# YooSungHyun/RNNTransducer

Hardware: AMD Instinct MI355X
Metric: utterances/sec (higher is better)
Workload: dtype f32

## Files before the change

### include/rnnt_hip.h

```cpp
#ifndef RNNT_HIP_H_
#define RNNT_HIP_H_

#include <stddef.h>
#include <stdint.h>

#ifdef __cplusplus
extern "C" {
#endif

#define RNNT_HIP_ABI_VERSION 4

#define RNNT_OK 0
#define RNNT_ERR_INVALID (-1)
#define RNNT_ERR_LAUNCH (-2)
#define RNNT_ERR_UNSUPPORTED (-3)
#define RNNT_ERR_TIMEOUT (-4)

int rnnt_hip_version(void);
const char* rnnt_hip_last_error(void);
int rnnt_hip_device_cus(void);

enum {
  RNNT_K_GEMM = 0,
  RNNT_K_LSTM_FWD = 1,
  RNNT_K_LSTM_BWD = 2,
  RNNT_K_LSE = 3,
  RNNT_K_ALPHABETA = 4,
  RNNT_K_LATGRAD = 5,
  RNNT_K_MISC = 6,
  RNNT_K_GEMM_HP = 7,
  RNNT_K_HP_SPLIT = 8,
  RNNT_K_COUNT = 9
};
int rnnt_hip_prof_enable(int on);
int rnnt_hip_prof_collect(double* ms, double* work, int64_t* count, int nkinds);

int rnnt_hip_lstm_launch_log_enable(int on);
int64_t rnnt_hip_lstm_launch_log(char* buf, size_t n);

#define RNNT_GEMM_GELU_A 1u
#define RNNT_GEMM_GELU_B 2u
#define RNNT_GEMM_ACCUM 4u
#define RNNT_GEMM_MUL_DGELU 8u
#define RNNT_GEMM_EXACT_F32 16u
#define RNNT_GEMM_HP_F16 32u

typedef struct rnnt_gemm_desc {
  int64_t M, N, K;
  const float* A;
  int64_t a_div, a_so, a_si, a_sk;
  int32_t a_mc;
  const int64_t* a_rowidx;
  const float* B;
  int64_t b_sn, b_sk;
  float* C;
  int64_t c_div, c_so, c_si;
  const float* bias;
  const float* aux;
  uint32_t flags;
  void* workspace;
  size_t workspace_bytes;
} rnnt_gemm_desc;

size_t rnnt_hip_gemm_workspace_bytes(int64_t M, int64_t N, int64_t K);
int rnnt_hip_gemm_f32(const rnnt_gemm_desc* d, void* stream);

size_t rnnt_hip_hp_bytes(int64_t rows, int64_t K);
int rnnt_hip_hp_split(const float* x, int64_t rows, int64_t K, int64_t ld, int32_t transpose, int64_t src_rows, int64_t shift,
                      void* planes, uint32_t* amax, int32_t amax_given, void* stream);
int rnnt_hip_hp_split_both(const float* x, int64_t M, int64_t C, int64_t ld, const uint32_t* rowmax, const uint32_t* colmax,
                           void* planes_rm, void* planes_t, void* stream);
size_t rnnt_hip_gemm_hp_workspace_bytes(int64_t M, int64_t N, int64_t K);
int rnnt_hip_gemm_hp(const void* A, const uint32_t* a_amax, const void* B, const uint32_t* b_amax, int64_t M, int64_t N, int64_t K,
                     float* C, int64_t ldc, const float* bias, uint32_t flags, void* workspace, size_t workspace_bytes,
                     void* stream);

typedef struct rnnt_hp_problem {
  const void* A; const uint32_t* a_amax;
  const void* B; const uint32_t* b_amax;
  int64_t M, N, K;
  float* C; int64_t ldc;
  uint32_t flags;
} rnnt_hp_problem;
size_t rnnt_hip_gemm_hp_grouped_workspace_bytes(const rnnt_hp_problem* problems, int32_t n);
int rnnt_hip_gemm_hp_grouped(const rnnt_hp_problem* problems, int32_t n, uint32_t xcd_skip, void* workspace, size_t workspace_bytes,
                             void* stream);

#define RNNT_CELL_LSTM 0
#define RNNT_CELL_GRU 1
#define RNNT_CELL_RNN_TANH 2
#define RNNT_CELL_RNN_RELU 3

typedef struct rnnt_lstm_desc {
  int32_t T, B, I, H, D;
  int32_t cell;
  const int32_t* lens;
  const float* x;
  int64_t x_st, x_sb;
  const float* w_ih[2];
  const float* w_hh[2];
  const float* b_ih[2];
  const float* b_hh[2];
  float* y;
  float* y_drop;
  float dropout_p;
  uint64_t dropout_seed;
  float* gates;
  float* cst;
  float* aux;
  void* workspace;
  size_t workspace_bytes;
  uint32_t* status;
  float x_abs_bound;
  const int32_t* row_idx;
  int32_t n_rows;
} rnnt_lstm_desc;

size_t rnnt_hip_lstm_workspace_bytes(int32_t T, int32_t B, int32_t I, int32_t H, int32_t D);
int32_t rnnt_hip_lstm_max_batch(int32_t H, int32_t D, int32_t cell);
int32_t rnnt_hip_lstm_free_xcds(int32_t T, int32_t B, int32_t H, int32_t D, int32_t cell);
int32_t rnnt_hip_lstm_takes_row_idx(int32_t T, int32_t B, int32_t I, int32_t H, int32_t D, int32_t cell);
int rnnt_hip_lstm_fwd(const rnnt_lstm_desc* d, void* stream);

#define RNNT_PRECISION_FP32 0
#define RNNT_PRECISION_F16 1
int rnnt_hip_lstm_fwd_ex(const rnnt_lstm_desc* d, uint32_t precision, void* stream);
int32_t rnnt_hip_lstm_takes_f16(int32_t T, int32_t B, int32_t I, int32_t H, int32_t D, int32_t cell);

typedef struct rnnt_lstm_bwd_desc {
  rnnt_lstm_desc f;
  const float* dy;
  float* dx;
  float* dw_ih[2];
  float* dw_hh[2];
  float* db[2];
  float* db_hh[2];
  int32_t accumulate;
  int32_t phase;
  int32_t beside_recurrence;
} rnnt_lstm_bwd_desc;
#define RNNT_LSTM_BWD_ALL 0
#define RNNT_LSTM_BWD_RECUR 1
#define RNNT_LSTM_BWD_WEIGHTS 2

int rnnt_hip_lstm_bwd(const rnnt_lstm_bwd_desc* d, void* stream);
int rnnt_hip_lstm_bwd_ex(const rnnt_lstm_bwd_desc* d, uint32_t precision, void* stream);
int rnnt_hip_lstm_check(const void* workspace, void* stream);
int rnnt_hip_lstm_debug_read(const void* workspace, int32_t T, int32_t B, int32_t I, int32_t H, int32_t D,
                             uint64_t* out, int32_t nwg, void* stream);

size_t rnnt_hip_joint_loss_workspace_bytes(int32_t B, int32_t T, int32_t U1, int32_t V);
int rnnt_hip_joint_loss_fwd_bwd(const float* A, int64_t a_sb, int64_t a_st, const float* C, int64_t c_sb, int64_t c_su,
                                const float* bias, const int32_t* labels, const int32_t* t_lens,
                                const int32_t* u_lens, int32_t B, int32_t T, int32_t U1, int32_t V, int32_t blank,
                                float gscale, float* nll, float* dA, float* dC, void* workspace,
                                size_t workspace_bytes, void* stream);

int rnnt_hip_joint_loss_bwd(const float* A, int64_t a_sb, int64_t a_st, const float* C, int64_t c_sb, int64_t c_su,
                            const float* bias, const int32_t* labels, const int32_t* t_lens, const int32_t* u_lens,
                            int32_t B, int32_t T, int32_t U1, int32_t V, int32_t blank, float gscale, const float* gvec,
                            int32_t gvec_stride, float* dA, float* dC, void* workspace, size_t workspace_bytes, void* stream);
int rnnt_hip_scaled_sum_f32(const float* x, int32_t n, float scale, float* out, void* stream);

int rnnt_hip_joint_logits_fwd(const float* A, int64_t a_sb, int64_t a_st, const float* C, int64_t c_sb, int64_t c_su,
                              const float* bias, int32_t B, int32_t T, int32_t U1, int32_t V, float* logits,
                              void* stream);

int rnnt_hip_loss_from_logits_fwd_bwd(const float* logits, const int32_t* labels, const int32_t* t_lens,
                                      const int32_t* u_lens, int32_t B, int32_t T, int32_t U1, int32_t V,
                                      int32_t blank, float gscale, float* nll, float* grad, void* workspace,
                                      size_t workspace_bytes, void* stream);

int rnnt_hip_embedding_fwd(const float* W, const int64_t* idx, int64_t M, int32_t H, int32_t V, float* out, void* stream);

#define RNNT_DTYPE_F32 0
#define RNNT_DTYPE_F16 1
#define RNNT_DTYPE_BF16 2
int rnnt_hip_loss_from_logits_fwd_bwd_ex(const void* logits, int32_t dtype, const int32_t* labels, const int32_t* t_lens,
                                         const int32_t* u_lens, int32_t B, int32_t T, int32_t U1, int32_t V, int32_t blank,
                                         float gscale, float* nll, void* grad, void* workspace, size_t workspace_bytes,
                                         void* stream);

int rnnt_hip_adamw_step(float* p, const float* g, float* m, float* v, int64_t n, float lr, float beta1, float beta2, float eps,
                        float weight_decay, int64_t step, void* stream);
int rnnt_hip_adamw_step_ex(float* p, const float* g, float* m, float* v, int64_t n, float lr, float beta1, float beta2, float eps,
                           float weight_decay, int64_t step, float grad_scale, const uint32_t* guard, void* stream);

size_t rnnt_hip_colsum_workspace_bytes(int64_t M, int64_t N);
int rnnt_hip_colsum_f32(const float* X, int64_t M, int64_t N, int64_t ld, float* out, void* workspace,
                        size_t workspace_bytes, void* stream);
int rnnt_hip_colsum_f32_acc(const float* X, int64_t M, int64_t N, int64_t ld, float* out, void* workspace,
                            size_t workspace_bytes, void* stream);

int rnnt_hip_embedding_bwd(const float* dE, const int64_t* idx, int64_t M, int32_t H, int32_t V, int64_t padding_idx,
                           float* dW, void* stream);
int rnnt_hip_embedding_bwd_acc(const float* dE, const int64_t* idx, int64_t M, int32_t H, int32_t V, int64_t padding_idx,
                               float* dW, void* stream);

#define RNNT_DECODE_MAX_LAYERS 8
typedef struct rnnt_decode_desc {
  int32_t T, B, V;
  int32_t Hp, O, L;
  int32_t cell;
  int32_t blank, max_iters, max_out;
  const float* A;
  const int32_t* t_lens;
  const float* emb;
  const float* w_ih[RNNT_DECODE_MAX_LAYERS];
  const float* w_hh[RNNT_DECODE_MAX_LAYERS];
  const float* b_ih[RNNT_DECODE_MAX_LAYERS];
  const float* b_hh[RNNT_DECODE_MAX_LAYERS];
  const float* w_o;
  const float* b_o;
  const float* w_d;
  int64_t ld_d;
  int64_t* tokens;
  int32_t* ntok;
} rnnt_decode_desc;
int rnnt_hip_greedy_decode(const rnnt_decode_desc* d, void* stream);

typedef struct rnnt_prednet_step_desc {
  int32_t B, Hp, L, cell;
  const int64_t* tokens;
  const float* emb;
  const float* w_ih[RNNT_DECODE_MAX_LAYERS];
  const float* w_hh[RNNT_DECODE_MAX_LAYERS];
  const float* b_ih[RNNT_DECODE_MAX_LAYERS];
  const float* b_hh[RNNT_DECODE_MAX_LAYERS];
  const float* h_in;
  const float* c_in;
  float* h_out;
  float* c_out;
} rnnt_prednet_step_desc;
int rnnt_hip_prednet_step(const rnnt_prednet_step_desc* d, void* stream);

#define RNNT_BEAM_ST_OK 0
#define RNNT_BEAM_ST_CANDIDATES 1
#define RNNT_BEAM_ST_POPS 2
#define RNNT_BEAM_ST_STATES 3
#define RNNT_BEAM_ST_NODES 4
#define RNNT_BEAM_ST_LEN 5
#define RNNT_BEAM_NSTATS 6
typedef struct rnnt_beam_desc {
  int32_t T, B, V;
  int32_t Hp, O, L;
  int32_t cell, blank;
  int32_t beam, improved;
  double state_beam, expand_beam;
  int32_t max_candidates, max_pops, max_states, max_nodes, max_len;
  const float* A;
  const int32_t* t_lens;
  const float* emb;
  const float* w_ih[RNNT_DECODE_MAX_LAYERS];
  const float* w_hh[RNNT_DECODE_MAX_LAYERS];
  const float* b_ih[RNNT_DECODE_MAX_LAYERS];
  const float* b_hh[RNNT_DECODE_MAX_LAYERS];
  const float* w_o;
  const float* b_o;
  const float* w_d;
  int64_t ld_d;
  void* workspace;
  size_t workspace_bytes;
  int32_t* tokens;
  int32_t* lens;
  double* scores;
  int32_t* count;
  int32_t* status;
  int32_t* stats;
} rnnt_beam_desc;
size_t rnnt_hip_beam_workspace_bytes(const rnnt_beam_desc* d);
int rnnt_hip_beam_search(const rnnt_beam_desc* d, void* stream);

#define RNNT_STREAM_MAX_LAYERS 8
typedef struct rnnt_stream_rnn_desc {
  int32_t T, B, F, H, L, cell;
  int32_t O, V;
  const float* x;
  int64_t x_sb, x_st;
  const int32_t* lens;
  const float* w_ih[RNNT_STREAM_MAX_LAYERS];
  const float* w_hh[RNNT_STREAM_MAX_LAYERS];
  const float* b_ih[RNNT_STREAM_MAX_LAYERS];
  const float* b_hh[RNNT_STREAM_MAX_LAYERS];
  float* h;
  float* c;
  const float* w_o;
  const float* b_o;
  float* out;
  int64_t out_sb, out_st;
  const float* fc_w;
  int64_t ld_fc;
  const float* fc_b;
  float* A;
  void* workspace;
  size_t workspace_bytes;
} rnnt_stream_rnn_desc;
size_t rnnt_hip_stream_rnn_workspace_bytes(const rnnt_stream_rnn_desc* d);
int rnnt_hip_stream_rnn_chunk(const rnnt_stream_rnn_desc* d, void* stream);

typedef struct rnnt_stream_greedy_desc {
  int32_t T, B, V, Hp, O, L, cell;
  int32_t blank, max_iters, max_out;
  const float* A;
  const int32_t* lens;
  const float* emb;
  const float* w_ih[RNNT_DECODE_MAX_LAYERS];
  const float* w_hh[RNNT_DECODE_MAX_LAYERS];
  const float* b_ih[RNNT_DECODE_MAX_LAYERS];
  const float* b_hh[RNNT_DECODE_MAX_LAYERS];
  const float* w_o;
  const float* b_o;
  const float* w_d;
  int64_t ld_d;
  float* h;
  float* c;
  float* C;
  int64_t* last;
  int64_t* tokens;
  int32_t* ntok;
} rnnt_stream_greedy_desc;
int rnnt_hip_stream_greedy(const rnnt_stream_greedy_desc* d, void* stream);
int rnnt_hip_stream_greedy_reset(const rnnt_stream_greedy_desc* d, const int32_t* rows, int32_t n_rows, void* stream);

typedef struct rnnt_beam_stream_desc {
  int32_t T, B, V;
  int32_t Hp, O, L;
  int32_t cell, blank;
  int32_t beam, improved;
  double state_beam, expand_beam;
  int32_t max_candidates, max_pops, max_states, max_nodes, max_len;
  const float* A;
  const int32_t* lens;
  const float* emb;
  const float* w_ih[RNNT_DECODE_MAX_LAYERS];
  const float* w_hh[RNNT_DECODE_MAX_LAYERS];
  const float* b_ih[RNNT_DECODE_MAX_LAYERS];
  const float* b_hh[RNNT_DECODE_MAX_LAYERS];
  const float* w_o;
  const float* b_o;
  const float* w_d;
  int64_t ld_d;
  void* workspace;
  size_t workspace_bytes;
  int32_t* tokens;
  int32_t* out_lens;
  double* scores;
  int32_t* count;
  int32_t* status;
  int32_t* commit;
  int32_t* ncommit;
  int32_t* stats;
} rnnt_beam_stream_desc;
size_t rnnt_hip_beam_stream_workspace_bytes(const rnnt_beam_stream_desc* d);
int rnnt_hip_beam_stream_reset(const rnnt_beam_stream_desc* d, const int32_t* rows, int32_t n_rows, int32_t build_table,
                               void* stream);
int rnnt_hip_beam_stream_chunk(const rnnt_beam_stream_desc* d, void* stream);

int rnnt_hip_frontend_norm_pad(const float* wav, int64_t ld, const int32_t* lens, int32_t B, int32_t pad, int64_t Lp,
                               int32_t normalize, float* out, void* stream);
int rnnt_hip_power_mel_log1p(const float* spec, int64_t M, int32_t n_bins, const float* fb, int32_t n_mels,
                             const int32_t* nframes, int32_t frames_per_utt, float* out, void* stream);

#ifdef __cplusplus
}
#endif
#endif
```

### rnntransducer_amd/_lib.py

```python
from __future__ import annotations

import ctypes as C
import os

_HERE = os.path.dirname(os.path.abspath(__file__))
LIB_PATH = os.environ.get("RNNT_HIP_LIB") or os.path.join(_HERE, "csrc", "librnnt_hip.so")
ABI_VERSION = 4

GEMM_GELU_A, GEMM_GELU_B, GEMM_ACCUM, GEMM_MUL_DGELU, GEMM_EXACT_F32 = 1, 2, 4, 8, 16
GEMM_HP_F16 = 32
PRECISION_FP32, PRECISION_F16 = 0, 1
CELL_LSTM, CELL_GRU, CELL_RNN_TANH, CELL_RNN_RELU = 0, 1, 2, 3

c_f32p = C.c_void_p
c_i64 = C.c_int64
c_i32 = C.c_int32


class GemmDesc(C.Structure):
    _fields_ = [("M", c_i64), ("N", c_i64), ("K", c_i64), ("A", C.c_void_p), ("a_div", c_i64), ("a_so", c_i64),
                ("a_si", c_i64), ("a_sk", c_i64), ("a_mc", c_i32), ("a_rowidx", C.c_void_p), ("B", C.c_void_p),
                ("b_sn", c_i64), ("b_sk", c_i64), ("C", C.c_void_p), ("c_div", c_i64), ("c_so", c_i64),
                ("c_si", c_i64), ("bias", C.c_void_p), ("aux", C.c_void_p), ("flags", C.c_uint32),
                ("workspace", C.c_void_p), ("workspace_bytes", C.c_size_t)]


class LstmDesc(C.Structure):
    _fields_ = [("T", c_i32), ("B", c_i32), ("I", c_i32), ("H", c_i32), ("D", c_i32), ("cell", c_i32), ("lens", C.c_void_p),
                ("x", C.c_void_p), ("x_st", c_i64), ("x_sb", c_i64), ("w_ih", C.c_void_p * 2),
                ("w_hh", C.c_void_p * 2), ("b_ih", C.c_void_p * 2), ("b_hh", C.c_void_p * 2), ("y", C.c_void_p),
                ("y_drop", C.c_void_p), ("dropout_p", C.c_float), ("dropout_seed", C.c_uint64),
                ("gates", C.c_void_p), ("cst", C.c_void_p), ("aux", C.c_void_p), ("workspace", C.c_void_p),
                ("workspace_bytes", C.c_size_t), ("status", C.c_void_p), ("x_abs_bound", C.c_float), ("row_idx", C.c_void_p),
                ("n_rows", c_i32)]


class LstmBwdDesc(C.Structure):
    _fields_ = [("f", LstmDesc), ("dy", C.c_void_p), ("dx", C.c_void_p), ("dw_ih", C.c_void_p * 2),
                ("dw_hh", C.c_void_p * 2), ("db", C.c_void_p * 2), ("db_hh", C.c_void_p * 2), ("accumulate", c_i32), ("phase", c_i32),
                ("beside_recurrence", c_i32)]


class HpProblem(C.Structure):
    _fields_ = [("A", C.c_void_p), ("a_amax", C.c_void_p), ("B", C.c_void_p), ("b_amax", C.c_void_p), ("M", c_i64), ("N", c_i64),
                ("K", c_i64), ("C", C.c_void_p), ("ldc", c_i64), ("flags", C.c_uint32)]


DECODE_MAX_LAYERS = 8


class DecodeDesc(C.Structure):
    _fields_ = [("T", c_i32), ("B", c_i32), ("V", c_i32), ("Hp", c_i32), ("O", c_i32), ("L", c_i32), ("cell", c_i32),
                ("blank", c_i32), ("max_iters", c_i32), ("max_out", c_i32), ("A", C.c_void_p), ("t_lens", C.c_void_p), ("emb", C.c_void_p),
                ("w_ih", C.c_void_p * DECODE_MAX_LAYERS), ("w_hh", C.c_void_p * DECODE_MAX_LAYERS),
                ("b_ih", C.c_void_p * DECODE_MAX_LAYERS), ("b_hh", C.c_void_p * DECODE_MAX_LAYERS),
                ("w_o", C.c_void_p), ("b_o", C.c_void_p), ("w_d", C.c_void_p), ("ld_d", c_i64),
                ("tokens", C.c_void_p), ("ntok", C.c_void_p)]


class PrednetStepDesc(C.Structure):
    _fields_ = [("B", c_i32), ("Hp", c_i32), ("L", c_i32), ("cell", c_i32), ("tokens", C.c_void_p), ("emb", C.c_void_p),
                ("w_ih", C.c_void_p * DECODE_MAX_LAYERS), ("w_hh", C.c_void_p * DECODE_MAX_LAYERS),
                ("b_ih", C.c_void_p * DECODE_MAX_LAYERS), ("b_hh", C.c_void_p * DECODE_MAX_LAYERS),
                ("h_in", C.c_void_p), ("c_in", C.c_void_p), ("h_out", C.c_void_p), ("c_out", C.c_void_p)]


BEAM_STATUS = {1: ("A entries in one frame", "max_candidates"), 2: ("pops in one frame", "max_pops"),
               3: ("live prediction-net states", "max_states"), 4: ("prefix-tree nodes", "max_nodes"),
               5: ("tokens in a returned hypothesis", "max_len")}
BEAM_NSTATS = 6


class BeamDesc(C.Structure):
    _fields_ = [("T", c_i32), ("B", c_i32), ("V", c_i32), ("Hp", c_i32), ("O", c_i32), ("L", c_i32), ("cell", c_i32),
                ("blank", c_i32), ("beam", c_i32), ("improved", c_i32), ("state_beam", C.c_double), ("expand_beam", C.c_double),
                ("max_candidates", c_i32), ("max_pops", c_i32), ("max_states", c_i32), ("max_nodes", c_i32), ("max_len", c_i32),
                ("A", C.c_void_p), ("t_lens", C.c_void_p), ("emb", C.c_void_p),
                ("w_ih", C.c_void_p * DECODE_MAX_LAYERS), ("w_hh", C.c_void_p * DECODE_MAX_LAYERS),
                ("b_ih", C.c_void_p * DECODE_MAX_LAYERS), ("b_hh", C.c_void_p * DECODE_MAX_LAYERS),
                ("w_o", C.c_void_p), ("b_o", C.c_void_p), ("w_d", C.c_void_p), ("ld_d", c_i64),
                ("workspace", C.c_void_p), ("workspace_bytes", C.c_size_t), ("tokens", C.c_void_p), ("lens", C.c_void_p),
                ("scores", C.c_void_p), ("count", C.c_void_p), ("status", C.c_void_p), ("stats", C.c_void_p)]


STREAM_MAX_LAYERS = 8


class StreamRnnDesc(C.Structure):
    _fields_ = [("T", c_i32), ("B", c_i32), ("F", c_i32), ("H", c_i32), ("L", c_i32), ("cell", c_i32), ("O", c_i32), ("V", c_i32),
                ("x", C.c_void_p), ("x_sb", c_i64), ("x_st", c_i64), ("lens", C.c_void_p),
                ("w_ih", C.c_void_p * STREAM_MAX_LAYERS), ("w_hh", C.c_void_p * STREAM_MAX_LAYERS),
                ("b_ih", C.c_void_p * STREAM_MAX_LAYERS), ("b_hh", C.c_void_p * STREAM_MAX_LAYERS),
                ("h", C.c_void_p), ("c", C.c_void_p), ("w_o", C.c_void_p), ("b_o", C.c_void_p),
                ("out", C.c_void_p), ("out_sb", c_i64), ("out_st", c_i64), ("fc_w", C.c_void_p), ("ld_fc", c_i64),
                ("fc_b", C.c_void_p), ("A", C.c_void_p), ("workspace", C.c_void_p), ("workspace_bytes", C.c_size_t)]


class StreamGreedyDesc(C.Structure):
    _fields_ = [("T", c_i32), ("B", c_i32), ("V", c_i32), ("Hp", c_i32), ("O", c_i32), ("L", c_i32), ("cell", c_i32),
                ("blank", c_i32), ("max_iters", c_i32), ("max_out", c_i32), ("A", C.c_void_p), ("lens", C.c_void_p),
                ("emb", C.c_void_p), ("w_ih", C.c_void_p * DECODE_MAX_LAYERS), ("w_hh", C.c_void_p * DECODE_MAX_LAYERS),
                ("b_ih", C.c_void_p * DECODE_MAX_LAYERS), ("b_hh", C.c_void_p * DECODE_MAX_LAYERS),
                ("w_o", C.c_void_p), ("b_o", C.c_void_p), ("w_d", C.c_void_p), ("ld_d", c_i64),
                ("h", C.c_void_p), ("c", C.c_void_p), ("C", C.c_void_p), ("last", C.c_void_p),
                ("tokens", C.c_void_p), ("ntok", C.c_void_p)]


class BeamStreamDesc(C.Structure):
    _fields_ = [("T", c_i32), ("B", c_i32), ("V", c_i32), ("Hp", c_i32), ("O", c_i32), ("L", c_i32), ("cell", c_i32),
                ("blank", c_i32), ("beam", c_i32), ("improved", c_i32), ("state_beam", C.c_double), ("expand_beam", C.c_double),
                ("max_candidates", c_i32), ("max_pops", c_i32), ("max_states", c_i32), ("max_nodes", c_i32), ("max_len", c_i32),
                ("A", C.c_void_p), ("lens", C.c_void_p), ("emb", C.c_void_p),
                ("w_ih", C.c_void_p * DECODE_MAX_LAYERS), ("w_hh", C.c_void_p * DECODE_MAX_LAYERS),
                ("b_ih", C.c_void_p * DECODE_MAX_LAYERS), ("b_hh", C.c_void_p * DECODE_MAX_LAYERS),
                ("w_o", C.c_void_p), ("b_o", C.c_void_p), ("w_d", C.c_void_p), ("ld_d", c_i64),
                ("workspace", C.c_void_p), ("workspace_bytes", C.c_size_t), ("tokens", C.c_void_p), ("out_lens", C.c_void_p),
                ("scores", C.c_void_p), ("count", C.c_void_p), ("status", C.c_void_p), ("commit", C.c_void_p),
                ("ncommit", C.c_void_p), ("stats", C.c_void_p)]


SYMBOLS = {
    "rnnt_hip_version": (C.c_int, []),
    "rnnt_hip_last_error": (C.c_char_p, []),
    "rnnt_hip_device_cus": (C.c_int, []),
    "rnnt_hip_prof_enable": (C.c_int, [C.c_int]),
    "rnnt_hip_prof_collect": (C.c_int, [C.c_void_p, C.c_void_p, C.c_void_p, C.c_int]),
    "rnnt_hip_lstm_launch_log_enable": (C.c_int, [C.c_int]),
    "rnnt_hip_lstm_launch_log": (c_i64, [C.c_char_p, C.c_size_t]),
    "rnnt_hip_gemm_workspace_bytes": (C.c_size_t, [c_i64, c_i64, c_i64]),
    "rnnt_hip_gemm_f32": (C.c_int, [C.POINTER(GemmDesc), C.c_void_p]),
    "rnnt_hip_hp_bytes": (C.c_size_t, [c_i64, c_i64]),
    "rnnt_hip_hp_split": (C.c_int, [C.c_void_p, c_i64, c_i64, c_i64, c_i32, c_i64, c_i64, C.c_void_p, C.c_void_p, c_i32, C.c_void_p]),
    "rnnt_hip_gemm_hp_workspace_bytes": (C.c_size_t, [c_i64, c_i64, c_i64]),
    "rnnt_hip_gemm_hp": (C.c_int, [C.c_void_p, C.c_void_p, C.c_void_p, C.c_void_p, c_i64, c_i64, c_i64, C.c_void_p, c_i64, C.c_void_p,
                                  C.c_uint32, C.c_void_p, C.c_size_t, C.c_void_p]),
    "rnnt_hip_hp_split_both": (C.c_int, [C.c_void_p, c_i64, c_i64, c_i64, C.c_void_p, C.c_void_p, C.c_void_p, C.c_void_p, C.c_void_p]),
    "rnnt_hip_gemm_hp_grouped_workspace_bytes": (C.c_size_t, [C.POINTER(HpProblem), c_i32]),
    "rnnt_hip_gemm_hp_grouped": (C.c_int, [C.POINTER(HpProblem), c_i32, C.c_uint32, C.c_void_p, C.c_size_t, C.c_void_p]),
    "rnnt_hip_lstm_workspace_bytes": (C.c_size_t, [c_i32] * 5),
    "rnnt_hip_lstm_max_batch": (c_i32, [c_i32, c_i32, c_i32]),
    "rnnt_hip_lstm_free_xcds": (c_i32, [c_i32] * 5),
    "rnnt_hip_lstm_takes_row_idx": (c_i32, [c_i32] * 6),
    "rnnt_hip_lstm_fwd": (C.c_int, [C.POINTER(LstmDesc), C.c_void_p]),
    "rnnt_hip_lstm_fwd_ex": (C.c_int, [C.POINTER(LstmDesc), C.c_uint32, C.c_void_p]),
    "rnnt_hip_lstm_takes_f16": (c_i32, [c_i32] * 6),
    "rnnt_hip_lstm_bwd": (C.c_int, [C.POINTER(LstmBwdDesc), C.c_void_p]),
    "rnnt_hip_lstm_bwd_ex": (C.c_int, [C.POINTER(LstmBwdDesc), C.c_uint32, C.c_void_p]),
    "rnnt_hip_lstm_check": (C.c_int, [C.c_void_p, C.c_void_p]),
    "rnnt_hip_lstm_debug_read": (C.c_int, [C.c_void_p, c_i32, c_i32, c_i32, c_i32, c_i32, C.c_void_p, c_i32, C.c_void_p]),
    "rnnt_hip_joint_loss_workspace_bytes": (C.c_size_t, [c_i32] * 4),
    "rnnt_hip_joint_loss_fwd_bwd": (C.c_int, [C.c_void_p, c_i64, c_i64, C.c_void_p, c_i64, c_i64, C.c_void_p, C.c_void_p,
                                               C.c_void_p, C.c_void_p, c_i32, c_i32, c_i32, c_i32, c_i32, C.c_float,
                                               C.c_void_p, C.c_void_p, C.c_void_p, C.c_void_p, C.c_size_t, C.c_void_p]),
    "rnnt_hip_joint_loss_bwd": (C.c_int, [C.c_void_p, c_i64, c_i64, C.c_void_p, c_i64, c_i64, C.c_void_p, C.c_void_p,
                                           C.c_void_p, C.c_void_p, c_i32, c_i32, c_i32, c_i32, c_i32, C.c_float, C.c_void_p, c_i32,
                                           C.c_void_p, C.c_void_p, C.c_void_p, C.c_size_t, C.c_void_p]),
    "rnnt_hip_scaled_sum_f32": (C.c_int, [C.c_void_p, c_i32, C.c_float, C.c_void_p, C.c_void_p]),
    "rnnt_hip_joint_logits_fwd": (C.c_int, [C.c_void_p, c_i64, c_i64, C.c_void_p, c_i64, c_i64, C.c_void_p, c_i32, c_i32,
                                             c_i32, c_i32, C.c_void_p, C.c_void_p]),
    "rnnt_hip_loss_from_logits_fwd_bwd": (C.c_int, [C.c_void_p, C.c_void_p, C.c_void_p, C.c_void_p, c_i32, c_i32, c_i32,
                                                     c_i32, c_i32, C.c_float, C.c_void_p, C.c_void_p, C.c_void_p,
                                                     C.c_size_t, C.c_void_p]),
    "rnnt_hip_loss_from_logits_fwd_bwd_ex": (C.c_int, [C.c_void_p, c_i32, C.c_void_p, C.c_void_p, C.c_void_p, c_i32, c_i32,
                                                        c_i32, c_i32, c_i32, C.c_float, C.c_void_p, C.c_void_p,
                                                        C.c_void_p, C.c_size_t, C.c_void_p]),
    "rnnt_hip_adamw_step": (C.c_int, [C.c_void_p, C.c_void_p, C.c_void_p, C.c_void_p, c_i64, C.c_float, C.c_float, C.c_float,
                                     C.c_float, C.c_float, c_i64, C.c_void_p]),
    "rnnt_hip_adamw_step_ex": (C.c_int, [C.c_void_p, C.c_void_p, C.c_void_p, C.c_void_p, c_i64, C.c_float, C.c_float, C.c_float,
                                        C.c_float, C.c_float, c_i64, C.c_float, C.c_void_p, C.c_void_p]),
    "rnnt_hip_embedding_fwd": (C.c_int, [C.c_void_p, C.c_void_p, c_i64, c_i32, c_i32, C.c_void_p, C.c_void_p]),
    "rnnt_hip_colsum_workspace_bytes": (C.c_size_t, [c_i64, c_i64]),
    "rnnt_hip_colsum_f32": (C.c_int, [C.c_void_p, c_i64, c_i64, c_i64, C.c_void_p, C.c_void_p, C.c_size_t, C.c_void_p]),
    "rnnt_hip_colsum_f32_acc": (C.c_int, [C.c_void_p, c_i64, c_i64, c_i64, C.c_void_p, C.c_void_p, C.c_size_t, C.c_void_p]),
    "rnnt_hip_embedding_bwd": (C.c_int, [C.c_void_p, C.c_void_p, c_i64, c_i32, c_i32, c_i64, C.c_void_p, C.c_void_p]),
    "rnnt_hip_embedding_bwd_acc": (C.c_int, [C.c_void_p, C.c_void_p, c_i64, c_i32, c_i32, c_i64, C.c_void_p, C.c_void_p]),
    "rnnt_hip_greedy_decode": (C.c_int, [C.POINTER(DecodeDesc), C.c_void_p]),
    "rnnt_hip_prednet_step": (C.c_int, [C.POINTER(PrednetStepDesc), C.c_void_p]),
    "rnnt_hip_beam_workspace_bytes": (C.c_size_t, [C.POINTER(BeamDesc)]),
    "rnnt_hip_beam_search": (C.c_int, [C.POINTER(BeamDesc), C.c_void_p]),
    "rnnt_hip_stream_rnn_workspace_bytes": (C.c_size_t, [C.POINTER(StreamRnnDesc)]),
    "rnnt_hip_stream_rnn_chunk": (C.c_int, [C.POINTER(StreamRnnDesc), C.c_void_p]),
    "rnnt_hip_stream_greedy": (C.c_int, [C.POINTER(StreamGreedyDesc), C.c_void_p]),
    "rnnt_hip_stream_greedy_reset": (C.c_int, [C.POINTER(StreamGreedyDesc), C.c_void_p, c_i32, C.c_void_p]),
    "rnnt_hip_beam_stream_workspace_bytes": (C.c_size_t, [C.POINTER(BeamStreamDesc)]),
    "rnnt_hip_beam_stream_reset": (C.c_int, [C.POINTER(BeamStreamDesc), C.c_void_p, c_i32, c_i32, C.c_void_p]),
    "rnnt_hip_beam_stream_chunk": (C.c_int, [C.POINTER(BeamStreamDesc), C.c_void_p]),
    "rnnt_hip_frontend_norm_pad": (C.c_int, [C.c_void_p, c_i64, C.c_void_p, c_i32, c_i32, c_i64, c_i32, C.c_void_p, C.c_void_p]),
    "rnnt_hip_power_mel_log1p": (C.c_int, [C.c_void_p, c_i64, c_i32, C.c_void_p, c_i32, C.c_void_p, c_i32, C.c_void_p, C.c_void_p]),
}

KERNEL_KINDS = ["gemm_f32_kernel", "lstm_fwd_kernel", "lstm_bwd_kernel", "lse_kernel", "alphabeta_kernel",
                "lattice_grad_kernel", "misc", "gemm_hp_kernel", "hp_split_kernels"]

_lib = None


class RnntHipError(RuntimeError):
    pass


def lib():
    global _lib
    if _lib is None:
        if not os.path.exists(LIB_PATH):
            raise RnntHipError(
                f"{LIB_PATH} not found: build it with `python -m rnntransducer_amd.csrc.build` "
                "(or __graft_entry__.build()).  rnntransducer_amd has no non-HIP execution path.")
        handle = C.CDLL(LIB_PATH)
        for name, (res, args) in SYMBOLS.items():
            fn = getattr(handle, name)
            fn.restype = res
            fn.argtypes = args
        if handle.rnnt_hip_version() != ABI_VERSION:
            raise RnntHipError(f"{LIB_PATH} reports ABI version {handle.rnnt_hip_version()}, this package binds version {ABI_VERSION}: "
                               "rebuild it with `python -m rnntransducer_amd.csrc.build`")
        _lib = handle
    return _lib


def check(rc: int, what: str = "") -> None:
    if rc != 0:
        msg = lib().rnnt_hip_last_error().decode("utf-8", "replace")
        if rc == -1:
            raise ValueError(f"{what}: {msg}")
        raise RnntHipError(f"{what}: rc={rc}: {msg}")
```

### rnntransducer_amd/csrc/common.hpp

```cpp
#pragma once
#include <hip/hip_runtime.h>
#include <stdarg.h>
#include <stdint.h>
#include <stdio.h>

#include <atomic>

#include "rnnt_hip.h"

namespace rnnt {

void set_error(const char* fmt, ...);

#define RNNT_CHECK_ARG(cond, ...)      \
  do {                                 \
    if (!(cond)) {                     \
      ::rnnt::set_error(__VA_ARGS__);  \
      return RNNT_ERR_INVALID;         \
    }                                  \
  } while (0)

#define RNNT_CHECK_HIP(expr)                                                          \
  do {                                                                                \
    hipError_t e_ = (expr);                                                           \
    if (e_ != hipSuccess) {                                                           \
      ::rnnt::set_error("%s failed: %s (%s:%d)", #expr, hipGetErrorString(e_), __FILE__, __LINE__); \
      return RNNT_ERR_LAUNCH;                                                         \
    }                                                                                 \
  } while (0)

#define RNNT_CHECK_LAUNCH() RNNT_CHECK_HIP(hipGetLastError())

struct ProfScope {
  ProfScope(int kind, double work, hipStream_t s);
  ~ProfScope();
  int kind_;
  double work_;
  hipStream_t stream_;
  void* start_;
};

extern std::atomic<bool> g_launch_log_on;
void launch_log_note(const void* kernel, hipStream_t s);

static inline int64_t ceil_div(int64_t a, int64_t b) { return (a + b - 1) / b; }

size_t hp_plane_bytes(int64_t rows, int64_t K);
int hp_colmax(const float* x, int64_t rows, int64_t C, int64_t ld, uint32_t* amax, hipStream_t s);
int hp_split(const float* x, int64_t rows, int64_t K, int64_t ld, uint32_t* amax, void* planes, hipStream_t s, const int* rowidx = nullptr);
int hp_split_t(const float* x, int64_t R, int64_t K, int64_t ld, int64_t Ksrc, int64_t shift, const uint32_t* amax, void* planes,
               hipStream_t s, const int* kidx = nullptr);
int hp_split_both(const float* x, int64_t M, int64_t C, int64_t ld, const uint32_t* rowmax, const uint32_t* colmax, void* planes_rm,
                  void* planes_t, hipStream_t s, const int* rowidx = nullptr);
size_t hp_gemm_workspace_bytes(int64_t M, int64_t N, int64_t K);
int hp_gemm(const void* A, const uint32_t* a_amax, const void* B, const uint32_t* b_amax, int64_t M, int64_t N, int64_t K, float* C,
            int64_t c_div, int64_t c_so, int64_t c_si, const float* bias, unsigned flags, void* workspace, size_t workspace_bytes,
            hipStream_t s, const int* a_rowidx = nullptr, int64_t a_plane_rows = 0, const int* c_rowidx = nullptr);
struct HpProblem {
  const void* A; const uint32_t* a_amax; const void* B; const uint32_t* b_amax;
  int64_t M, N, K;
  float* C; int64_t ldc;
  unsigned flags;
};
constexpr int HP_GROUP_MAX = 4;
size_t hp_gemm_grouped_workspace_bytes(const int64_t* MN, int n);
int hp_gemm_grouped(const HpProblem* pr, int n, unsigned xcd_skip, unsigned* counter, void* workspace, size_t workspace_bytes,
                    hipStream_t s, unsigned* status = nullptr);
constexpr size_t HPQ_HEADER_BYTES = 256;
static inline size_t align_up(size_t a, size_t b) { return (a + b - 1) / b * b; }

__device__ __forceinline__ float gelu_tanh(float x) {
  const float k0 = 0.7978845608028654f, k1 = 0.044715f;
  float u = k0 * (x + k1 * x * x * x);
  return 0.5f * x * (1.0f + tanhf(u));
}
__device__ __forceinline__ float dgelu_tanh(float x) {
  const float k0 = 0.7978845608028654f, k1 = 0.044715f;
  float x2 = x * x;
  float u = k0 * (x + k1 * x * x2);
  float th = tanhf(u);
  float du = k0 * (1.0f + 3.0f * k1 * x2);
  return 0.5f * (1.0f + th) + 0.5f * x * (1.0f - th * th) * du;
}

__device__ __forceinline__ float sigmoidf_(float x) { return 1.0f / (1.0f + expf(-x)); }
__device__ __forceinline__ float tanh_e(float x) { return 1.0f - 2.0f / (expf(2.0f * x) + 1.0f); }
__device__ __forceinline__ float sigmoid_hw(float x) { return __builtin_amdgcn_rcpf(1.0f + __expf(-x)); }
__device__ __forceinline__ float tanh_hw(float x) { return 1.0f - 2.0f * __builtin_amdgcn_rcpf(__expf(2.0f * x) + 1.0f); }

typedef float f32x4 __attribute__((ext_vector_type(4)));
typedef float f32x16 __attribute__((ext_vector_type(16)));
typedef __bf16 bf16x8 __attribute__((ext_vector_type(8)));
typedef unsigned u32x4 __attribute__((ext_vector_type(4)));
typedef unsigned u32x2 __attribute__((ext_vector_type(2)));

template <int NPL>
__device__ __forceinline__ void split_pair(float xe, float xo, unsigned (&pk)[NPL]) {
  constexpr unsigned SEL = 0x07060302u;
  const unsigned ue = __float_as_uint(xe), uo = __float_as_uint(xo);
  pk[0] = __builtin_amdgcn_perm(uo, ue, SEL);
  const float re = xe - __uint_as_float(ue & 0xffff0000u), ro = xo - __uint_as_float(uo & 0xffff0000u);
  unsigned ure = __float_as_uint(re), uro = __float_as_uint(ro);
  if constexpr (NPL == 2) {
    ure += 0x8000u;
    uro += 0x8000u;
  }
  pk[1] = __builtin_amdgcn_perm(uro, ure, SEL);
  if constexpr (NPL == 3) {
    const float le = re - __uint_as_float(ure & 0xffff0000u), lo = ro - __uint_as_float(uro & 0xffff0000u);
    pk[2] = __builtin_amdgcn_perm(__float_as_uint(lo), __float_as_uint(le), SEL);
  }
}

__device__ __forceinline__ void split8(const f32x4& lo4, const f32x4& hi4, bf16x8 (&piece)[3]) {
  unsigned q0[3], q1[3], q2[3], q3[3];
  split_pair<3>(lo4[0], lo4[1], q0);
  split_pair<3>(lo4[2], lo4[3], q1);
  split_pair<3>(hi4[0], hi4[1], q2);
  split_pair<3>(hi4[2], hi4[3], q3);
#pragma unroll
  for (int pl = 0; pl < 3; ++pl) piece[pl] = __builtin_bit_cast(bf16x8, (u32x4){q0[pl], q1[pl], q2[pl], q3[pl]});
}

}
```

### rnntransducer_amd/csrc/gemm_hp.hip

```cpp
#include "common.hpp"

#include <stdlib.h>

namespace rnnt {
namespace {

typedef _Float16 f16x8 __attribute__((ext_vector_type(8)));
typedef __attribute__((address_space(3))) void lds_void;

constexpr int HP_BM = 256, HP_BN = 256, HP_BK = 32;
constexpr int HP_STAGE = (HP_BM + HP_BN) * 128;
constexpr int HP_RSRC = 0x00027000;

__device__ __forceinline__ float hp_scale_from_amax(unsigned amax_bits) {
  int eb = (int)((amax_bits >> 23) & 255u);
  if (eb == 0) return 1.0f;
  eb = eb < 15 ? 15 : eb;
  return __uint_as_float((unsigned)(268 - eb) << 23);
}
__device__ __forceinline__ float hp_inv_scale_from_amax(unsigned amax_bits) {
  int eb = (int)((amax_bits >> 23) & 255u);
  if (eb == 0) return 1.0f;
  eb = eb < 15 ? 15 : eb;
  return __uint_as_float((unsigned)(eb - 14) << 23);
}

__global__ void __launch_bounds__(256) hp_colmax_kernel(const float* __restrict__ x, long rows, int C, long ld, long rows_per_chunk,
                                                        unsigned* __restrict__ out) {
  const int c = blockIdx.x * 256 + threadIdx.x;
  if (c >= C) return;
  const long r0 = (long)blockIdx.y * rows_per_chunk, r1 = min(rows, r0 + rows_per_chunk);
  unsigned m = 0;
  for (long r = r0; r < r1; ++r) m = max(m, __float_as_uint(x[r * ld + c]) & 0x7fffffffu);
  if (m != 0) atomicMax(out + c, m);
}

__device__ __forceinline__ void hp_split8(const float (&x)[8], float scale, u32x4& hi, u32x4& lo) {
  f16x8 h, l;
#pragma unroll
  for (int e = 0; e < 8; ++e) {
    const float v = x[e] * scale;
    const _Float16 a = (_Float16)v;
    h[e] = a;
    l[e] = (_Float16)(v - (float)a);
  }
  hi = __builtin_bit_cast(u32x4, h);
  lo = __builtin_bit_cast(u32x4, l);
}

__global__ void __launch_bounds__(256) hp_split_kernel(const float* __restrict__ x, long rows, int K, long ld, unsigned* __restrict__ amax,
                                                       char* __restrict__ out, const int* __restrict__ rowidx) {
  const int Kp = (K + 31) & ~31, cpr = Kp >> 3;
  const int lane = threadIdx.x & 63;
  const bool vec = (ld & 3) == 0 && (reinterpret_cast<uintptr_t>(x) & 15) == 0;
  for (long ri = (long)blockIdx.x * 4 + (threadIdx.x >> 6); ri < rows; ri += (long)gridDim.x * 4) {
    const long r = rowidx ? (long)rowidx[ri] : ri;
    const float* row = x + r * ld;
    unsigned m = 0;
    for (int c = lane; c < cpr; c += 64) {
      const int k = 8 * c;
      if (vec && k + 7 < K) {
        const u32x4 a = *reinterpret_cast<const u32x4*>(row + k), b = *reinterpret_cast<const u32x4*>(row + k + 4);
#pragma unroll
        for (int e = 0; e < 4; ++e) m = max(m, max(a[e] & 0x7fffffffu, b[e] & 0x7fffffffu));
      } else {
#pragma unroll
        for (int e = 0; e < 8; ++e)
          if (k + e < K) m = max(m, __float_as_uint(row[k + e]) & 0x7fffffffu);
      }
    }
#pragma unroll
    for (int o = 32; o > 0; o >>= 1) m = max(m, (unsigned)__shfl_xor((int)m, o));
    if (lane == 0) amax[r] = m;
    const float scale = hp_scale_from_amax(m);
    for (int c = lane; c < cpr; c += 64) {
      const int k = 8 * c;
      float v[8];
      if (vec && k + 7 < K) {
        const f32x4 a = *reinterpret_cast<const f32x4*>(row + k), b = *reinterpret_cast<const f32x4*>(row + k + 4);
        v[0] = a[0]; v[1] = a[1]; v[2] = a[2]; v[3] = a[3]; v[4] = b[0]; v[5] = b[1]; v[6] = b[2]; v[7] = b[3];
      } else {
#pragma unroll
        for (int e = 0; e < 8; ++e) v[e] = (k + e < K) ? row[k + e] : 0.f;
      }
      u32x4 hi, lo;
      hp_split8(v, scale, hi, lo);
      char* dst = out + (r * (Kp >> 5) + (c >> 2)) * 128 + 16 * (c & 3);
      *reinterpret_cast<u32x4*>(dst) = hi;
      *reinterpret_cast<u32x4*>(dst + 64) = lo;
    }
  }
}

__global__ void __launch_bounds__(256) hp_split_t_kernel(const float* __restrict__ x, int R, int K, long ld, int Ksrc, int shift,
                                                         const unsigned* __restrict__ amax, char* __restrict__ out,
                                                         const int* __restrict__ kidx) {
  __shared__ float tile[32][257];
  const int kb = blockIdx.x, r0 = blockIdx.y * 256;
  const int tid = threadIdx.x;
  const bool vec = (ld & 3) == 0 && (reinterpret_cast<uintptr_t>(x) & 15) == 0;
#pragma unroll
  for (int q = 0; q < 8; ++q) {
    const int kk = 4 * q + (tid >> 6);
    const int kdst = kb * 32 + kk;
    const int ksrc = (kidx ? (kdst < K ? kidx[kdst] : 0) : kdst) + shift;
    const int c = 4 * (tid & 63);
    f32x4 v = {0.f, 0.f, 0.f, 0.f};
    if (kdst < K && ksrc >= 0 && ksrc < Ksrc) {
      const float* src = x + (long)ksrc * ld + r0 + c;
      if (vec && r0 + c + 3 < R) {
        v = *reinterpret_cast<const f32x4*>(src);
      } else {
#pragma unroll
        for (int e = 0; e < 4; ++e)
          if (r0 + c + e < R) v[e] = src[e];
      }
    }
#pragma unroll
    for (int e = 0; e < 4; ++e) tile[kk][c + e] = v[e];
  }
  __syncthreads();
  const int Kp32 = (K + 31) >> 5;
#pragma unroll
  for (int ps = 0; ps < 4; ++ps) {
    const int rl = (tid >> 2) + 64 * ps, ch = tid & 3;
    if (r0 + rl < R) {
      float v[8];
#pragma unroll
      for (int e = 0; e < 8; ++e) v[e] = tile[8 * ch + e][rl];
      u32x4 hi, lo;
      hp_split8(v, hp_scale_from_amax(amax[r0 + rl]), hi, lo);
      char* dst = out + ((long)(r0 + rl) * Kp32 + kb) * 128 + 16 * ch;
      *reinterpret_cast<u32x4*>(dst) = hi;
      *reinterpret_cast<u32x4*>(dst + 64) = lo;
    }
  }
}

__global__ void __launch_bounds__(256) hp_split_both_kernel(const float* __restrict__ x, int M, int C, long ld, const unsigned* __restrict__ rowmax,
                                                            const unsigned* __restrict__ colmax, char* __restrict__ out_rm, char* __restrict__ out_t,
                                                            const int* __restrict__ rowidx) {
  __shared__ float tile[32][257];
  const int kb = blockIdx.x, c0 = blockIdx.y * 256;
  const int tid = threadIdx.x;
  const int Cp = (C + 31) & ~31;
  const bool vec = (ld & 3) == 0 && (reinterpret_cast<uintptr_t>(x) & 15) == 0;
#pragma unroll
  for (int q = 0; q < 4; ++q) {
    const int row = 8 * q + (tid >> 5), col = 8 * (tid & 31);
    const int ri = kb * 32 + row, c = c0 + col;
    const int r = (rowidx && ri < M) ? rowidx[ri] : ri;
    float v[8] = {0.f, 0.f, 0.f, 0.f, 0.f, 0.f, 0.f, 0.f};
    if (ri < M && c < C) {
      const float* src = x + (long)r * ld + c;
      if (vec && c + 7 < C) {
        const f32x4 a = *reinterpret_cast<const f32x4*>(src), b = *reinterpret_cast<const f32x4*>(src + 4);
        v[0] = a[0]; v[1] = a[1]; v[2] = a[2]; v[3] = a[3]; v[4] = b[0]; v[5] = b[1]; v[6] = b[2]; v[7] = b[3];
      } else {
#pragma unroll
        for (int e = 0; e < 8; ++e)
          if (c + e < C) v[e] = src[e];
      }
    }
    if (ri < M && c < Cp) {
      u32x4 hi, lo;
      hp_split8(v, hp_scale_from_amax(rowmax[r]), hi, lo);
      char* dst = out_rm + ((long)r * (Cp >> 5) + (c >> 5)) * 128 + 16 * ((c >> 3) & 3);
      *reinterpret_cast<u32x4*>(dst) = hi;
      *reinterpret_cast<u32x4*>(dst + 64) = lo;
    }
#pragma unroll
    for (int e = 0; e < 8; ++e) tile[row][col + e] = v[e];
  }
  __syncthreads();
  const int Mp32 = (M + 31) >> 5;
#pragma unroll
  for (int ps = 0; ps < 4; ++ps) {
    const int rl = (tid >> 2) + 64 * ps, ch = tid & 3;
    if (c0 + rl < C) {
      float v[8];
#pragma unroll
      for (int e = 0; e < 8; ++e) v[e] = tile[8 * ch + e][rl];
      u32x4 hi, lo;
      hp_split8(v, hp_scale_from_amax(colmax[c0 + rl]), hi, lo);
      char* dst = out_t + ((long)(c0 + rl) * Mp32 + kb) * 128 + 16 * ch;
      *reinterpret_cast<u32x4*>(dst) = hi;
      *reinterpret_cast<u32x4*>(dst + 64) = lo;
    }
  }
}

struct HpGemmK {
  int M, N, nkt;
  const char* A; unsigned a_pitch, a_bytes;
  const char* B; unsigned b_pitch, b_bytes;
  const unsigned* a_amax; const unsigned* b_amax;
  float* C; int c_div; long c_so, c_si;
  const float* bias;
  unsigned flags;
  int splits, kt_per_split;
  float* slab;
  int tiles_m, tiles_n;
  int group_m;
  const int* a_rowidx;
  const int* c_rowidx;
};

__device__ __forceinline__ int hp_xcd_remap(int bid, int n) {
  const int q = n / 8, r = n % 8, xcd = bid % 8;
  return (xcd < r ? xcd * (q + 1) : r * (q + 1) + (xcd - r) * q) + bid / 8;
}

template <bool F16>
__device__ __forceinline__ void hp_tile256(const HpGemmK& p, const int bid, const int z, char* lds) {
  const int tid = threadIdx.x, lane = tid & 63;
  const int wave = __builtin_amdgcn_readfirstlane(tid >> 6);
  const int wr = wave >> 2, wc = wave & 3;
  const int m0 = (bid % p.tiles_m) * HP_BM, n0 = (bid / p.tiles_m) * HP_BN;

  const __amdgpu_buffer_rsrc_t ra = __builtin_amdgcn_make_buffer_rsrc(const_cast<char*>(p.A), 0, (int)p.a_bytes, HP_RSRC);
  const __amdgpu_buffer_rsrc_t rb = __builtin_amdgcn_make_buffer_rsrc(const_cast<char*>(p.B), 0, (int)p.b_bytes, HP_RSRC);

  unsigned va[4], vb[4];
  {
    const int src_slot = (lane & 7) ^ (((lane >> 4) & 3) | ((wave & 1) << 2));
#pragma unroll
    for (int j = 0; j < 4; ++j) {
      const int row = (8 * j + wave) * 8 + (lane >> 3);
      int ma = min(m0 + row, p.M - 1);
      const int nb = min(n0 + row, p.N - 1);
      if (p.a_rowidx) ma = p.a_rowidx[ma];
      va[j] = (unsigned)ma * p.a_pitch + 16u * src_slot;
      vb[j] = (unsigned)nb * p.b_pitch + 16u * src_slot;
    }
  }
  auto stage = [&](int buf, int kt) {
    char* base = lds + buf * HP_STAGE;
    const int koff = kt * 128;
#pragma unroll
    for (int j = 0; j < 4; ++j) {
      __builtin_amdgcn_raw_ptr_buffer_load_lds(ra, (lds_void*)(base + (8 * j + wave) * 1024), 16, va[j], koff, 0, 0);
      __builtin_amdgcn_raw_ptr_buffer_load_lds(rb, (lds_void*)(base + HP_BM * 128 + (8 * j + wave) * 1024), 16, vb[j], koff, 0, 0);
    }
  };

  const int frag0 = (lane & 15) * 128 + 16 * ((lane >> 4) ^ ((lane & 15) >> 1));
  const int a_base = wr * (128 * 128) + frag0;
  const int b_base = HP_BM * 128 + wc * (64 * 128) + frag0;

  f32x4 acc[8][4];
#pragma unroll
  for (int i = 0; i < 8; ++i)
#pragma unroll
    for (int j = 0; j < 4; ++j) acc[i][j] = (f32x4){0.f, 0.f, 0.f, 0.f};

  const int kt0 = z * p.kt_per_split;
  const int nk = min(p.nkt - kt0, p.kt_per_split);

  stage(0, kt0);
  asm volatile("s_waitcnt vmcnt(0)" ::: "memory");
  __syncthreads();
  for (int kt = 0; kt < nk; ++kt) {
    const int cur = kt & 1;
#ifndef HP_DBG_NO_DMA
    if (kt + 1 < nk) stage(cur ^ 1, kt0 + kt + 1);
#endif
    const char* sb = lds + cur * HP_STAGE;
    f16x8 a[4][2], b[2][2];
#ifdef HP_DBG_NO_LDSREAD
    auto load_a = [&](int mq) {
#pragma unroll
      for (int i = 0; i < 4; ++i) { asm volatile("" : "+v"(a[i][0]), "+v"(a[i][1])); }
    };
    auto load_b = [&](int nq) {
#pragma unroll
      for (int j = 0; j < 2; ++j) { asm volatile("" : "+v"(b[j][0]), "+v"(b[j][1])); }
    };
#else
    auto load_a = [&](int mq) {
#pragma unroll
      for (int i = 0; i < 4; ++i) {
        a[i][0] = *reinterpret_cast<const f16x8*>(sb + (a_base + (4 * mq + i) * 2048));
        if constexpr (!F16) a[i][1] = *reinterpret_cast<const f16x8*>(sb + ((a_base ^ 64) + (4 * mq + i) * 2048));
      }
    };
    auto load_b = [&](int nq) {
#pragma unroll
      for (int j = 0; j < 2; ++j) {
        b[j][0] = *reinterpret_cast<const f16x8*>(sb + (b_base + (2 * nq + j) * 2048));
        if constexpr (!F16) b[j][1] = *reinterpret_cast<const f16x8*>(sb + ((b_base ^ 64) + (2 * nq + j) * 2048));
      }
    };
#endif
    auto mma = [&](int mq, int nq) {
#pragma unroll
      for (int i = 0; i < 4; ++i)
#pragma unroll
        for (int j = 0; j < 2; ++j) {
          f32x4 c = acc[4 * mq + i][2 * nq + j];
          if constexpr (!F16) {
            c = __builtin_amdgcn_mfma_f32_16x16x32_f16(a[i][1], b[j][0], c, 0, 0, 0);
            c = __builtin_amdgcn_mfma_f32_16x16x32_f16(a[i][0], b[j][1], c, 0, 0, 0);
          }
          c = __builtin_amdgcn_mfma_f32_16x16x32_f16(a[i][0], b[j][0], c, 0, 0, 0);
          acc[4 * mq + i][2 * nq + j] = c;
        }
    };
#ifndef HP_DBG_NO_MFMA
    load_a(0); load_b(0); mma(0, 0);
    load_b(1); mma(0, 1);
    load_a(1); mma(1, 1);
    load_b(0); mma(1, 0);
#endif
    __builtin_amdgcn_sched_barrier(0);
#ifndef HP_DBG_NO_BARRIER
    __syncthreads();
#endif
  }
  const int mode = p.splits > 1 ? 0 : ((p.flags & RNNT_GEMM_ACCUM) ? 2 : 1);
  float* slab = p.splits > 1 ? p.slab + (long)z * p.M * p.N : nullptr;
  float bias_v[4], sb[4];
#pragma unroll
  for (int j = 0; j < 4; ++j) {
    const int n = n0 + wc * 64 + j * 16 + (lane & 15);
    bias_v[j] = (mode != 0 && p.bias && n < p.N) ? p.bias[n] : 0.f;
    sb[j] = hp_inv_scale_from_amax(p.b_amax[min(n, p.N - 1)]);
  }
#pragma unroll
  for (int i = 0; i < 8; ++i) {
#pragma unroll
    for (int reg = 0; reg < 4; ++reg) {
      const int m = m0 + wr * 128 + i * 16 + 4 * (lane >> 4) + reg;
      const bool mok = m < p.M;
      const int mc = mok ? m : 0;
      const float sa = hp_inv_scale_from_amax(p.a_amax[p.a_rowidx ? p.a_rowidx[mc] : mc]);
      const int mo = p.c_rowidx ? p.c_rowidx[mc] : mc;
      float* crow = mode == 0 ? slab + (long)mc * p.N : p.C + (long)(mo / p.c_div) * p.c_so + (long)(mo % p.c_div) * p.c_si;
      float old[4] = {0.f, 0.f, 0.f, 0.f};
      if (mode == 2) {
#pragma unroll
        for (int j = 0; j < 4; ++j) {
          const int n = n0 + wc * 64 + j * 16 + (lane & 15);
          if (mok && n < p.N) old[j] = crow[n];
        }
      }
#pragma unroll
      for (int j = 0; j < 4; ++j) {
        const int n = n0 + wc * 64 + j * 16 + (lane & 15);
        if (mok && n < p.N) crow[n] = acc[i][j][reg] * sa * sb[j] + bias_v[j] + old[j];
      }
    }
  }
}

__device__ __forceinline__ int hp_grouped_tile(int idx, int tiles_m, int tiles_n, int group_m) {
  const int band = group_m * tiles_n;
  const int g = idx / band, r = idx - g * band;
  const int m_first = g * group_m;
  const int gm = min(tiles_m - m_first, group_m);
  const int n = r / gm, m = m_first + (r - n * gm);
  return n * tiles_m + m;
}

template <bool F16>
__global__ void __launch_bounds__(512, 1) gemm_hp_kernel(const HpGemmK p) {
  extern __shared__ __attribute__((aligned(16))) char lds[];
  int bid = hp_xcd_remap(blockIdx.x, p.tiles_m * p.tiles_n);
  if (p.group_m > 0) bid = hp_grouped_tile(bid, p.tiles_m, p.tiles_n, p.group_m);
  hp_tile256<F16>(p, bid, blockIdx.y, lds);
}

constexpr int HPQ_MAX = 4;
struct HpGemmQ {
  HpGemmK prob[HPQ_MAX];
  int unit_end[HPQ_MAX];
  int nprob;
  unsigned xcd_skip;
  unsigned* counter;
};

template <bool F16>
__global__ void __launch_bounds__(512, 1) gemm_hpq_kernel(const HpGemmQ q) {
  extern __shared__ __attribute__((aligned(16))) char lds[];
  unsigned xcc;
  asm volatile("s_getreg_b32 %0, hwreg(HW_REG_XCC_ID)" : "=s"(xcc));
  xcc &= 7u;
  if ((q.xcd_skip >> xcc) & 1u) return;
  const unsigned allow = ~q.xcd_skip & 0xffu;
  const int nq = __builtin_popcount(allow);
  const int mine = __builtin_popcount(allow & ((1u << xcc) - 1u));
  int* next = reinterpret_cast<int*>(lds + 2 * HP_STAGE);
  const int total = q.unit_end[q.nprob - 1];
  for (int hop = 0; hop < nq; ++hop) {
    const int qi = (mine + hop) % nq;
    const int lo = (int)((long)total * qi / nq), hi = (int)((long)total * (qi + 1) / nq);
    while (true) {
      if (threadIdx.x == 0) {
        const int got = lo + (int)atomicAdd(q.counter + qi, 1u);
        *next = got;
        if (got < hi) atomicAdd(q.counter + 8, 1u);
      }
      __syncthreads();
      const int u = __builtin_amdgcn_readfirstlane(*next);
      __syncthreads();
      if (u >= hi) break;
      int pi = 0;
      while (u >= q.unit_end[pi]) ++pi;
      const HpGemmK& p = q.prob[pi];
      const int local = u - (pi ? q.unit_end[pi - 1] : 0);
      const int tn = local % p.tiles_n, z = (local / p.tiles_n) % p.splits, tm = local / (p.tiles_n * p.splits);
      hp_tile256<F16>(p, tn * p.tiles_m + tm, z, lds);
    }
  }
}

__global__ void hpq_check_kernel(unsigned* counter, unsigned total, unsigned* status) {
  if (counter[8] != total) {
    counter[9] = 1u;
    if (status) __hip_atomic_store(status, 2u, __ATOMIC_RELAXED, __HIP_MEMORY_SCOPE_AGENT);
  }
}

__global__ void __launch_bounds__(256) hp_splitk_reduce_kernel(const HpGemmK p) {
  const long total = (long)p.M * p.N;
  for (long i = (long)blockIdx.x * 256 + threadIdx.x; i < total; i += (long)gridDim.x * 256) {
    const int m = (int)(i / p.N), n = (int)(i % p.N);
    float s = 0.f;
    for (int z = 0; z < p.splits; ++z) s += p.slab[(long)z * total + i];
    if (p.bias) s += p.bias[n];
    const int mo = p.c_rowidx ? p.c_rowidx[m] : m;
    const long off = (long)(mo / p.c_div) * p.c_so + (long)(mo % p.c_div) * p.c_si + n;
    if (p.flags & RNNT_GEMM_ACCUM) s += p.C[off];
    p.C[off] = s;
  }
}

}

size_t hp_plane_bytes(int64_t rows, int64_t K) { return (size_t)rows * (size_t)ceil_div(K, 32) * 128; }

int hp_colmax(const float* x, int64_t rows, int64_t C, int64_t ld, uint32_t* amax, hipStream_t s) {
  RNNT_CHECK_HIP(hipMemsetAsync(amax, 0, (size_t)C * 4, s));
  if (rows == 0 || C == 0) return RNNT_OK;
  long chunks = ceil_div(2048, ceil_div(C, 256));
  if (chunks > ceil_div(rows, 64)) chunks = ceil_div(rows, 64);
  if (chunks < 1) chunks = 1;
  const long rpc = ceil_div(rows, chunks);
  ProfScope prof(RNNT_K_HP_SPLIT, 4.0 * (double)rows * (double)C, s);
  hipLaunchKernelGGL(hp_colmax_kernel, dim3((unsigned)ceil_div(C, 256), (unsigned)ceil_div(rows, rpc)), dim3(256), 0, s, x, (long)rows, (int)C,
                     (long)ld, rpc, amax);
  RNNT_CHECK_LAUNCH();
  return RNNT_OK;
}

int hp_split(const float* x, int64_t rows, int64_t K, int64_t ld, uint32_t* amax, void* planes, hipStream_t s, const int* rowidx) {
  if (rows == 0) return RNNT_OK;
  const long blocks = ceil_div(rows, 4);
  ProfScope prof(RNNT_K_HP_SPLIT, 8.0 * (double)rows * (double)K, s);
  hipLaunchKernelGGL(hp_split_kernel, dim3((unsigned)(blocks < 8192 ? blocks : 8192)), dim3(256), 0, s, x, (long)rows, (int)K, (long)ld, amax,
                     (char*)planes, rowidx);
  RNNT_CHECK_LAUNCH();
  return RNNT_OK;
}

int hp_split_t(const float* x, int64_t R, int64_t K, int64_t ld, int64_t Ksrc, int64_t shift, const uint32_t* amax, void* planes,
               hipStream_t s, const int* kidx) {
  if (R == 0 || K == 0) return RNNT_OK;
  ProfScope prof(RNNT_K_HP_SPLIT, 8.0 * (double)R * (double)K, s);
  hipLaunchKernelGGL(hp_split_t_kernel, dim3((unsigned)ceil_div(K, 32), (unsigned)ceil_div(R, 256)), dim3(256), 0, s, x, (int)R, (int)K, (long)ld,
                     (int)Ksrc, (int)shift, amax, (char*)planes, kidx);
  RNNT_CHECK_LAUNCH();
  return RNNT_OK;
}

int hp_split_both(const float* x, int64_t M, int64_t C, int64_t ld, const uint32_t* rowmax, const uint32_t* colmax, void* planes_rm,
                  void* planes_t, hipStream_t s, const int* rowidx) {
  if (M == 0 || C == 0) return RNNT_OK;
  ProfScope prof(RNNT_K_HP_SPLIT, 12.0 * (double)M * (double)C, s);
  hipLaunchKernelGGL(hp_split_both_kernel, dim3((unsigned)ceil_div(M, 32), (unsigned)ceil_div(C, 256)), dim3(256), 0, s, x, (int)M, (int)C, (long)ld,
                     rowmax, colmax, (char*)planes_rm, (char*)planes_t, rowidx);
  RNNT_CHECK_LAUNCH();
  return RNNT_OK;
}

size_t hp_gemm_workspace_bytes(int64_t M, int64_t N, int64_t K) {
  const long tiles = ceil_div(M, HP_BM) * ceil_div(N, HP_BN);
  const long nkt = ceil_div(K, HP_BK);
  if (tiles >= 192 || nkt < 64) return 0;
  long want = ceil_div(256, tiles);
  if (want > nkt / 32) want = nkt / 32;
  if (want > 32) want = 32;
  return want >= 2 ? (size_t)want * M * N * 4 : 0;
}

int hp_gemm(const void* A, const uint32_t* a_amax, const void* B, const uint32_t* b_amax, int64_t M, int64_t N, int64_t K, float* C,
            int64_t c_div, int64_t c_so, int64_t c_si, const float* bias, unsigned flags, void* workspace, size_t workspace_bytes,
            hipStream_t s, const int* a_rowidx, int64_t a_plane_rows, const int* c_rowidx) {
  RNNT_CHECK_ARG(A && B && C && a_amax && b_amax, "gemm_hp: null operand");
  RNNT_CHECK_ARG(!a_rowidx || a_plane_rows >= M, "gemm_hp: a gathered A operand needs the row count of its planes");
  RNNT_CHECK_ARG(M >= 1 && N >= 1 && K >= 1 && M < (1ll << 31) && N < (1ll << 31) && K < (1ll << 31), "gemm_hp: bad dims");
  RNNT_CHECK_ARG(c_div >= 1, "gemm_hp: c_div must be >= 1");
  RNNT_CHECK_ARG(((reinterpret_cast<uintptr_t>(A) | reinterpret_cast<uintptr_t>(B)) & 127) == 0, "gemm_hp: planes must be 128-byte aligned");
  HpGemmK k;
  k.M = (int)M; k.N = (int)N; k.nkt = (int)ceil_div(K, HP_BK);
  const size_t ab = hp_plane_bytes(a_rowidx ? a_plane_rows : M, K), bb = hp_plane_bytes(N, K);
  RNNT_CHECK_ARG(ab < (1ull << 32) && bb < (1ull << 32), "gemm_hp: an operand exceeds the 4 GB a buffer resource addresses");
  k.A = (const char*)A; k.a_pitch = (unsigned)k.nkt * 128u; k.a_bytes = (unsigned)ab;
  k.B = (const char*)B; k.b_pitch = (unsigned)k.nkt * 128u; k.b_bytes = (unsigned)bb;
  k.a_amax = a_amax; k.b_amax = b_amax;
  k.C = C; k.c_div = (int)(c_div > 0x7fffffff ? 0x7fffffff : c_div); k.c_so = c_so; k.c_si = c_si;
  k.bias = bias; k.flags = flags;
  k.a_rowidx = a_rowidx; k.c_rowidx = c_rowidx;
  const bool f16 = (flags & RNNT_GEMM_HP_F16) != 0u;
  k.tiles_m = (int)ceil_div(M, HP_BM); k.tiles_n = (int)ceil_div(N, HP_BN);
  const int tiles = k.tiles_m * k.tiles_n;
  {
    static const int env_gm = getenv("RNNT_GEMM_HP_GROUP_M") ? atoi(getenv("RNNT_GEMM_HP_GROUP_M")) : -1;
    k.group_m = env_gm >= 0 ? env_gm : (tiles >= 256 ? 8 : 4);
  }
  int splits = 1;
  if (workspace && tiles < 192 && k.nkt >= 64) {
    long want = ceil_div(256, tiles);
    const long by_ws = (long)(workspace_bytes / ((size_t)M * N * 4));
    if (want > k.nkt / 32) want = k.nkt / 32;
    if (want > by_ws) want = by_ws;
    if (want > 32) want = 32;
    if (want >= 2) splits = (int)want;
  }
  k.kt_per_split = (int)ceil_div(k.nkt, splits);
  splits = (int)ceil_div(k.nkt, k.kt_per_split);
  k.splits = splits;
  k.slab = (float*)workspace;
  if (f16) RNNT_CHECK_HIP(hipFuncSetAttribute((const void*)gemm_hp_kernel<true>, hipFuncAttributeMaxDynamicSharedMemorySize, 2 * HP_STAGE));
  else RNNT_CHECK_HIP(hipFuncSetAttribute((const void*)gemm_hp_kernel<false>, hipFuncAttributeMaxDynamicSharedMemorySize, 2 * HP_STAGE));
  {
    ProfScope prof(RNNT_K_GEMM_HP, 2.0 * (double)M * (double)N * (double)K, s);
    if (f16) hipLaunchKernelGGL(gemm_hp_kernel<true>, dim3(tiles, splits), dim3(512), 2 * HP_STAGE, s, k);
    else hipLaunchKernelGGL(gemm_hp_kernel<false>, dim3(tiles, splits), dim3(512), 2 * HP_STAGE, s, k);
    RNNT_CHECK_LAUNCH();
    if (splits > 1) {
      const long blocks = ceil_div((long)M * N, 256);
      hipLaunchKernelGGL(hp_splitk_reduce_kernel, dim3((unsigned)(blocks < 2048 ? blocks : 2048)), dim3(256), 0, s, k);
      RNNT_CHECK_LAUNCH();
    }
  }
  return RNNT_OK;
}

constexpr int HPQ_SPLIT_CAP = 8;
size_t hp_gemm_grouped_workspace_bytes(const int64_t* MN, int n) {
  size_t total = 0;
  for (int i = 0; i < n; ++i) total += align_up((size_t)HPQ_SPLIT_CAP * (size_t)MN[i] * 4, 256);
  return total;
}

int hp_gemm_grouped(const HpProblem* pr, int n, unsigned xcd_skip, unsigned* counter, void* workspace, size_t workspace_bytes,
                    hipStream_t s, unsigned* status) {
  RNNT_CHECK_ARG(pr && n >= 1 && n <= HPQ_MAX && counter, "gemm_hp grouped: 1..%d problems and a counter word", HPQ_MAX);
  RNNT_CHECK_ARG((xcd_skip & 0xffu) != 0xffu, "gemm_hp grouped: xcd_skip leaves no XCD");
  const bool f16 = (pr[0].flags & RNNT_GEMM_HP_F16) != 0u;
  for (int i = 1; i < n; ++i)
    RNNT_CHECK_ARG(((pr[i].flags & RNNT_GEMM_HP_F16) != 0u) == f16, "gemm_hp grouped: the problems of one launch share RNNT_GEMM_HP_F16");
  HpGemmQ q = {};
  q.nprob = n; q.xcd_skip = xcd_skip; q.counter = counter;
  int xcds = 0;
  for (int x = 0; x < 8; ++x) xcds += !((xcd_skip >> x) & 1u);
  const long workers = 32l * xcds;
  long total_kt = 0;
  double flops = 0.0;
  for (int i = 0; i < n; ++i) {
    const HpProblem& a = pr[i];
    RNNT_CHECK_ARG(a.A && a.B && a.C && a.a_amax && a.b_amax, "gemm_hp grouped: null operand (problem %d)", i);
    RNNT_CHECK_ARG(a.M >= 1 && a.N >= 1 && a.K >= 1 && a.M < (1ll << 31) && a.N < (1ll << 31) && a.K < (1ll << 31) && a.ldc >= a.N,
                   "gemm_hp grouped: bad dims (problem %d)", i);
    RNNT_CHECK_ARG(((reinterpret_cast<uintptr_t>(a.A) | reinterpret_cast<uintptr_t>(a.B)) & 127) == 0, "gemm_hp grouped: planes must be 128-byte aligned");
    HpGemmK& k = q.prob[i];
    k.M = (int)a.M; k.N = (int)a.N; k.nkt = (int)ceil_div(a.K, HP_BK);
    const size_t ab = hp_plane_bytes(a.M, a.K), bb = hp_plane_bytes(a.N, a.K);
    RNNT_CHECK_ARG(ab < (1ull << 32) && bb < (1ull << 32), "gemm_hp grouped: an operand exceeds the 4 GB a buffer resource addresses");
    k.A = (const char*)a.A; k.a_pitch = (unsigned)k.nkt * 128u; k.a_bytes = (unsigned)ab;
    k.B = (const char*)a.B; k.b_pitch = (unsigned)k.nkt * 128u; k.b_bytes = (unsigned)bb;
    k.a_amax = a.a_amax; k.b_amax = a.b_amax;
    k.C = a.C; k.c_div = 1; k.c_so = a.ldc; k.c_si = 0;
    k.bias = nullptr; k.flags = a.flags;
    k.a_rowidx = k.c_rowidx = nullptr;
    k.tiles_m = (int)ceil_div(a.M, HP_BM); k.tiles_n = (int)ceil_div(a.N, HP_BN);
    total_kt += (long)k.tiles_m * k.tiles_n * k.nkt;
    flops += 2.0 * (double)a.M * (double)a.N * (double)a.K;
  }
  long chunk = ceil_div(total_kt, 4 * workers);
  if (chunk < 32) chunk = 32;
  size_t off = 0;
  int units = 0;
  for (int i = 0; i < n; ++i) {
    HpGemmK& k = q.prob[i];
    long splits = ceil_div(k.nkt, chunk);
    if (splits > HPQ_SPLIT_CAP) splits = HPQ_SPLIT_CAP;
    const size_t per = (size_t)k.M * k.N * 4;
    while (splits > 1 && (!workspace || off + align_up((size_t)splits * per, 256) > workspace_bytes)) --splits;
    k.kt_per_split = (int)ceil_div(k.nkt, splits);
    k.splits = (int)ceil_div(k.nkt, k.kt_per_split);
    k.slab = k.splits > 1 ? reinterpret_cast<float*>((char*)workspace + off) : nullptr;
    if (k.splits > 1) off += align_up((size_t)k.splits * per, 256);
    units += k.tiles_m * k.tiles_n * k.splits;
    q.unit_end[i] = units;
  }
  RNNT_CHECK_HIP(hipMemsetAsync(counter, 0, 64, s));
  const int lds = 2 * HP_STAGE + 16;
  const void* qk = f16 ? (const void*)gemm_hpq_kernel<true> : (const void*)gemm_hpq_kernel<false>;
  RNNT_CHECK_HIP(hipFuncSetAttribute(qk, hipFuncAttributeMaxDynamicSharedMemorySize, lds));
  {
    ProfScope prof(RNNT_K_GEMM_HP, flops, s);
    int cus = 0, dev = 0;
    if (hipGetDevice(&dev) != hipSuccess || hipDeviceGetAttribute(&cus, hipDeviceAttributeMultiprocessorCount, dev) != hipSuccess || cus < 8) cus = 256;
    const dim3 grid(!xcd_skip && units < cus ? units : cus);
    if (f16) hipLaunchKernelGGL(gemm_hpq_kernel<true>, grid, dim3(512), lds, s, q);
    else hipLaunchKernelGGL(gemm_hpq_kernel<false>, grid, dim3(512), lds, s, q);
    RNNT_CHECK_LAUNCH();
    hipLaunchKernelGGL(hpq_check_kernel, dim3(1), dim3(1), 0, s, counter, (unsigned)units, status);
    RNNT_CHECK_LAUNCH();
    for (int i = 0; i < n; ++i)
      if (q.prob[i].splits > 1) {
        const long blocks = ceil_div((long)q.prob[i].M * q.prob[i].N, 256);
        hipLaunchKernelGGL(hp_splitk_reduce_kernel, dim3((unsigned)(blocks < 2048 ? blocks : 2048)), dim3(256), 0, s, q.prob[i]);
        RNNT_CHECK_LAUNCH();
      }
  }
  return RNNT_OK;
}

}

using namespace rnnt;

extern "C" size_t rnnt_hip_hp_bytes(int64_t rows, int64_t K) {
  if (rows < 0 || K < 0) return 0;
  return hp_plane_bytes(rows, K);
}

extern "C" int rnnt_hip_hp_split(const float* x, int64_t rows, int64_t K, int64_t ld, int32_t transpose, int64_t src_rows, int64_t shift,
                                 void* planes, uint32_t* amax, int32_t amax_given, void* stream) {
  RNNT_CHECK_ARG(x && planes && amax && rows >= 0 && K >= 0, "hp_split: bad arguments");
  RNNT_CHECK_ARG((reinterpret_cast<uintptr_t>(planes) & 127) == 0, "hp_split: planes must be 128-byte aligned");
  hipStream_t s = (hipStream_t)stream;
  if (!transpose) {
    RNNT_CHECK_ARG(ld >= K, "hp_split: ld < K");
    RNNT_CHECK_ARG(!amax_given, "hp_split: the row-major split computes its row maxima itself");
    return hp_split(x, rows, K, ld, amax, planes, s);
  }
  RNNT_CHECK_ARG(ld >= rows && src_rows >= 1, "hp_split: transposed source is (src_rows x >= rows), ld >= rows");
  if (!amax_given)
    if (int rc = hp_colmax(x, src_rows, rows, ld, amax, s)) return rc;
  return hp_split_t(x, rows, K, ld, src_rows, shift, amax, planes, s);
}

extern "C" size_t rnnt_hip_gemm_hp_workspace_bytes(int64_t M, int64_t N, int64_t K) {
  if (M < 1 || N < 1 || K < 1) return 0;
  return hp_gemm_workspace_bytes(M, N, K);
}

extern "C" int rnnt_hip_gemm_hp(const void* A, const uint32_t* a_amax, const void* B, const uint32_t* b_amax, int64_t M, int64_t N,
                                int64_t K, float* C, int64_t ldc, const float* bias, uint32_t flags, void* workspace,
                                size_t workspace_bytes, void* stream) {
  RNNT_CHECK_ARG(ldc >= N, "gemm_hp: ldc < N");
  return hp_gemm(A, a_amax, B, b_amax, M, N, K, C, 1, ldc, 0, bias, flags, workspace, workspace_bytes, (hipStream_t)stream);
}

static_assert(sizeof(rnnt_hp_problem) == sizeof(HpProblem), "rnnt_hp_problem mirrors HpProblem");

extern "C" size_t rnnt_hip_gemm_hp_grouped_workspace_bytes(const rnnt_hp_problem* problems, int32_t n) {
  if (!problems || n < 1 || n > HP_GROUP_MAX) return 0;
  int64_t mn[HP_GROUP_MAX];
  for (int i = 0; i < n; ++i) mn[i] = problems[i].M * problems[i].N;
  return 256 + hp_gemm_grouped_workspace_bytes(mn, n);
}

extern "C" int rnnt_hip_gemm_hp_grouped(const rnnt_hp_problem* problems, int32_t n, uint32_t xcd_skip, void* workspace,
                                        size_t workspace_bytes, void* stream) {
  RNNT_CHECK_ARG(problems && n >= 1 && n <= HP_GROUP_MAX, "gemm_hp grouped: 1..%d problems", HP_GROUP_MAX);
  RNNT_CHECK_ARG(workspace && workspace_bytes >= 256 && (reinterpret_cast<uintptr_t>(workspace) & 255) == 0,
                 "gemm_hp grouped: workspace of >= 256 bytes, 256-byte aligned");
  HpProblem pr[HP_GROUP_MAX];
  for (int i = 0; i < n; ++i) {
    const rnnt_hp_problem& a = problems[i];
    pr[i] = HpProblem{a.A, a.a_amax, a.B, a.b_amax, a.M, a.N, a.K, a.C, a.ldc, a.flags};
  }
  return hp_gemm_grouped(pr, n, xcd_skip, reinterpret_cast<unsigned*>(workspace), (char*)workspace + 256, workspace_bytes - 256,
                         (hipStream_t)stream);
}

extern "C" int rnnt_hip_hp_split_both(const float* x, int64_t M, int64_t C, int64_t ld, const uint32_t* rowmax, const uint32_t* colmax,
                                      void* planes_rm, void* planes_t, void* stream) {
  RNNT_CHECK_ARG(x && rowmax && colmax && planes_rm && planes_t && M >= 0 && C >= 0 && ld >= C, "hp_split_both: bad arguments");
  RNNT_CHECK_ARG(M < (1ll << 31) && C < (1ll << 31), "hp_split_both: dims must fit 31 bits");
  RNNT_CHECK_ARG(((reinterpret_cast<uintptr_t>(planes_rm) | reinterpret_cast<uintptr_t>(planes_t)) & 127) == 0, "hp_split_both: planes must be 128-byte aligned");
  return hp_split_both(x, M, C, ld, rowmax, colmax, planes_rm, planes_t, (hipStream_t)stream);
}
```

### rnntransducer_amd/csrc/lstm.hip

```cpp
#include "lstm_shared.hpp"

#include <string.h>

namespace rnnt {
namespace {

template <int MT, int NT>
__global__ void __launch_bounds__(256) lstm_fwd_kernel(const LstmK p) {
  extern __shared__ __attribute__((aligned(16))) char smem[];
  float* Wl = reinterpret_cast<float*>(smem);
  f32x4* part = reinterpret_cast<f32x4*>(Wl + 4 * p.Hs * p.LDW);
  int* abort_lds = reinterpret_cast<int*>(part + 4 * MT * NT * 64);

  const int tid = threadIdx.x, lane = tid & 63, wave = tid >> 6;
  const int n = lane & 15, q = lane >> 4;
  const int d = blockIdx.x / p.NC, wg = blockIdx.x % p.NC;
  const int H = p.H, B = p.B, D = p.D, T = p.T, Bp = p.Bp, LDW = p.LDW;
  const int j0 = wg * p.Hs;
  const int R = 4 * p.Hs;

  {
    const float* W = p.w_hh[d];
    for (int idx = tid; idx < R * LDW; idx += 256) {
      const int r = idx / LDW, k = idx % LDW;
// ... 1287 lines not shown

bool make_plan(int B, int H, int D, int cus, Plan* pl) {
  if (H < 4 || H % 4 != 0 || B < 1 || B > 64 || D < 1 || D > 2) return false;
  const int NT = B <= 16 ? 1 : (B <= 32 ? 2 : 4);
  pl->NT = NT;
  pl->Bp = 16 * NT;
  const int KG = (H + 15) / 16;
  pl->LDW = 16 * KG + 4;
  for (int per_cu = 1; per_cu <= 2; ++per_cu) {
    for (int Hs = 4; Hs <= 16; Hs *= 2) {
      if (H % Hs != 0) continue;
      const int MT = Hs / 4, NC = H / Hs;
      if (MT * NT > 4) continue;
      const size_t lds_fwd = (size_t)4 * Hs * pl->LDW * 4 + (size_t)4 * MT * NT * 64 * 16 + 16;
      const size_t lds_bwd = (size_t)KG * MT * 64 * 16 + (size_t)16 * MT * 4 * NT * 16 * 4 + 16;
      const size_t lds = lds_fwd > lds_bwd ? lds_fwd : lds_bwd;
      if (lds * per_cu > 160 * 1024) continue;
      if ((long)D * NC > (long)cus * per_cu) continue;
      pl->Hs = Hs; pl->NC = NC; pl->MT = MT; pl->wgs_per_cu = per_cu;
      pl->lds_fwd = lds_fwd; pl->lds_bwd = lds_bwd;
      return true;
    }
  }
  return false;
}


bool make_plan2(int B, int H, int D, int cus, Plan2* pl) {
  if (H < 4 || H % 4 != 0 || B < 1 || D < 1 || D > 2) return false;
  if (getenv("RNNT_LSTM_V1")) return false;
  const int Kp = (int)align_up((size_t)H, 64);
  for (int HS = 16; HS >= 4; HS /= 2) {
    if (H % HS != 0) continue;
    const int NC = H / HS;
    const int Gmax = cus / (D * NC);
    if (Gmax < 1) continue;
    int G = (int)ceil_div(B, 4);
    if (G > Gmax) G = Gmax;
    const int Bg = (int)ceil_div(B, G);
    if (Bg > 16) continue;
    G = (int)ceil_div(B, Bg);
    const int BQ = Bg <= 4 ? 1 : (Bg <= 8 ? 2 : 4);
    const int KSf = 16 / HS, KSb = 64 / HS;
    const size_t wa = (size_t)16 * Kp * HS;
    const size_t part = (size_t)4 * BQ * 64 * 16;
    const size_t lds_f = wa + (size_t)4 * (1024 + 4 * BQ * KSf * 4) * 4 + part + 16;
    const size_t lds_b = wa + (size_t)4 * (1024 + 4 * BQ * KSb * 4) * 4 + part + 16;
    if (lds_f > 160 * 1024 || lds_b > 160 * 1024) continue;
    pl->HS = HS; pl->NC = NC; pl->G = G; pl->Bg = Bg; pl->BQ = BQ; pl->Kp = Kp;
    pl->lds_fwd = lds_f; pl->lds_bwd = lds_b;
    return true;
  }
  return false;
}

bool make_plan3(int B, int H, int D, int cus, bool bwd, Plan2* pl) {
  if (getenv("RNNT_LSTM_V1") || getenv("RNNT_LSTM_V2")) return false;
  if (H % 128 != 0 || B < 1 || D < 1 || D > 2) return false;
  const int nks = H / 128;
  if (!(nks >= 1 && nks <= 6) && nks != 8) return false;
  (void)bwd;
  const bool h640 = nks == 5;
  const int MB = h640 ? 5 : 4, HS = 4 * MB;
  const int NC = H / HS;
  const int Gmax = cus / (D * NC);
  if (Gmax < 1) return false;
  int G = (int)ceil_div(B, 4);
  if (G > Gmax) G = Gmax;
  const int Bg = (int)ceil_div(B, G);
  if (Bg > 16) return false;
  G = (int)ceil_div(B, Bg);
  pl->HS = HS; pl->NC = NC; pl->G = G; pl->Bg = Bg; pl->BQ = Bg <= 4 ? 1 : (Bg <= 8 ? 2 : 4);
  pl->Kp = h640 ? 768 : H;
  pl->MB = MB;
  const int nwv = (nks >= 6 || h640) ? 8 : 4;
  const int ksb = (16 * MB + 31) / 32;
  pl->lds_fwd = (size_t)nwv * MB * 64 * 16 + 16;
  pl->lds_bwd = (size_t)nwv * 64 * 16 + 16 * (32 * ksb + 4) * 4 + 16;
  return true;
}

LstmWs carve_lstm(void* ws, int T, int B, int I, int H, int D, const Plan& pl) {
  LstmWs w;
  char* p = reinterpret_cast<char*>(ws);
  size_t off = 0;
  auto take = [&](size_t bytes) { char* q = p ? p + off : nullptr; off += align_up(bytes, 256); return q; };
  size_t nflags = (size_t)D * pl.NC;
  size_t hxb = (size_t)2 * D * H * pl.Bp * 4 * 4;
  {
    Plan2 p2;
    int cus = device_cus();
    if (cus <= 0) cus = 256;
    if (make_plan2(B, H, D, cus, &p2)) {
      const size_t nf2 = (size_t)D * p2.G * p2.NC;
      const size_t hx2 = (size_t)2 * D * p2.G * 4 * p2.BQ * 4 * p2.Kp * 4;
      if (nf2 > nflags) nflags = nf2;
      if (hx2 > hxb) hxb = hx2;
    }
    for (int bwd = 0; bwd < 2; ++bwd) {
      if (!make_plan3(B, H, D, cus, bwd != 0, &p2)) continue;
      const size_t nf3 = (size_t)D * p2.G * p2.NC;
      const size_t hx3 = bwd ? (size_t)2 * D * p2.G * p2.NC * 4 * p2.BQ * p2.Kp * 4
                             : (size_t)2 * D * p2.G * 4 * p2.BQ * p2.Kp * 6;
      if (nf3 > nflags) nflags = nf3;
      if (hx3 > hxb) hxb = hx3;
    }
  }
  w.nflags = nflags;
  w.sync_bytes = align_up((2 * nflags + 16) * 4, 16);
  w.flags = reinterpret_cast<unsigned*>(take(w.sync_bytes));
  w.hx_bytes = hxb;
  w.hx = reinterpret_cast<float*>(take(w.hx_bytes));
  w.wp = reinterpret_cast<float*>(take((size_t)D * 4 * H * I * 4));
  w.bp = reinterpret_cast<float*>(take((size_t)D * 4 * H * 4));
  w.dwhh = reinterpret_cast<float*>(take((size_t)D * 4 * H * H * 4));
  w.dbg = reinterpret_cast<unsigned long long*>(take(512 * 8 * 8));
  w.dbp_half = (size_t)D * (B + 64) * 4 * H;
  w.dbp = reinterpret_cast<float*>(take(2 * w.dbp_half * 4));
  {
    const int64_t M = (int64_t)T * B, N4 = (int64_t)D * 4 * H;
    size_t sc = rnnt_hip_gemm_workspace_bytes(N4, I, M);
    const size_t s2 = rnnt_hip_gemm_workspace_bytes(4 * H, H, M > B ? M - B : 1);
    const size_t s3 = rnnt_hip_colsum_workspace_bytes(M, N4);
    if (s2 > sc) sc = s2;
    if (s3 > sc) sc = s3;
    w.hp = use_hp(T, B, I, H, D);
    if (w.hp) {
      const size_t h1 = hp_gemm_workspace_bytes(N4, I, M), h2 = hp_gemm_workspace_bytes(4 * H, H, M);
      if (h1 > sc) sc = h1;
      if (h2 > sc) sc = h2;
      const int64_t mn[3] = {N4 * I, (int64_t)4 * H * H, (int64_t)4 * H * H};
      const size_t h3 = HPQ_HEADER_BYTES + hp_gemm_grouped_workspace_bytes(mn, 1 + D);
      if (h3 > sc) sc = h3;
    }
    w.scratch_bytes = sc;
    w.scratch = take(sc);
    w.hp_x = w.hp_w = w.hp_dg = w.hp_dgt = w.hp_yt = nullptr;
    w.hp_amax = nullptr;
    if (w.hp) {
      w.hp_amax = reinterpret_cast<uint32_t*>(take((size_t)(2 * M + 3 * N4 + 2 * I + (int64_t)D * H) * 4));
      w.hp_x = take(hp_plane_bytes(M, I) > hp_plane_bytes(I, M) ? hp_plane_bytes(M, I) : hp_plane_bytes(I, M));
      w.hp_w = take(hp_plane_bytes(N4, I) > hp_plane_bytes(I, N4) ? hp_plane_bytes(N4, I) : hp_plane_bytes(I, N4));
      w.hp_dg = take(hp_plane_bytes(M, N4));
      w.hp_dgt = take(hp_plane_bytes(N4, M));
      w.hp_yt = take((size_t)D * hp_plane_bytes(H, M));
    }
  }
  w.total = off;
  return w;
}

template <typename K>
int launch_persistent(K kernel, const LstmK& k, const Plan& pl, size_t lds, hipStream_t s, const char* what) {
  if (lds > 64 * 1024)
    RNNT_CHECK_HIP(hipFuncSetAttribute((const void*)kernel, hipFuncAttributeMaxDynamicSharedMemorySize, (int)lds));
  int per_cu = 0;
  RNNT_CHECK_HIP(hipOccupancyMaxActiveBlocksPerMultiprocessor(&per_cu, kernel, 256, lds));
  const int cus = device_cus();
  if (per_cu < 1 || (long)k.D * k.NC > (long)cus * (per_cu < pl.wgs_per_cu ? per_cu : pl.wgs_per_cu)) {
    set_error("%s: %d workgroups cannot be co-resident (%d CUs x %d per CU)", what, k.D * k.NC, cus, per_cu);
    return RNNT_ERR_UNSUPPORTED;
  }
  {
    const double per_tb = (k.dy ? (8.0 + 2.0 + 1.0) : (8.0 + 1.0 + 1.0)) * k.H * 4.0;
    ProfScope prof(k.dy ? RNNT_K_LSTM_BWD : RNNT_K_LSTM_FWD,
                   per_tb * k.T * k.B * k.D + 4.0 * 4.0 * k.H * k.H * k.D, s);
    hipLaunchKernelGGL(kernel, dim3(k.D * k.NC), dim3(256), lds, s, k);
  }
  RNNT_CHECK_LAUNCH();
  if (g_launch_log_on.load(std::memory_order_relaxed)) launch_log_note((const void*)kernel, s);
  return RNNT_OK;
}

int check_desc(const rnnt_lstm_desc* d, Plan* pl, LstmWs* w) {
  RNNT_CHECK_ARG(d != nullptr, "lstm: null descriptor");
  RNNT_CHECK_ARG(d->T >= 1 && d->I >= 1, "lstm: T and I must be positive (T=%d I=%d)", d->T, d->I);
  const int cus = device_cus();
  RNNT_CHECK_ARG(cus > 0, "lstm: no HIP device");
  if (!make_plan(d->B, d->H, d->D, cus, pl)) {
    set_error("lstm: unsupported configuration B=%d H=%d D=%d (need H%%4==0, 1<=B<=64, D in {1,2}, slice must fit %d CUs)",
              d->B, d->H, d->D, cus);
    return RNNT_ERR_UNSUPPORTED;
  }
  RNNT_CHECK_ARG(d->cell >= RNNT_CELL_LSTM && d->cell <= RNNT_CELL_RNN_RELU, "lstm: unknown cell type %d", d->cell);
  RNNT_CHECK_ARG(d->lens && d->x && d->y && d->gates && (d->cst || d->cell != RNNT_CELL_LSTM), "lstm: null tensor");
  for (int k = 0; k < d->D; ++k)
    RNNT_CHECK_ARG(d->w_ih[k] && d->w_hh[k] && d->b_ih[k] && d->b_hh[k], "lstm: null weight (direction %d)", k);
  RNNT_CHECK_ARG(d->dropout_p >= 0.f && d->dropout_p < 1.f, "lstm: dropout_p must be in [0,1)");
  RNNT_CHECK_ARG(d->dropout_p == 0.f || d->y_drop, "lstm: dropout_p > 0 needs y_drop");
  RNNT_CHECK_ARG(d->x_abs_bound >= 0.f && d->x_abs_bound < 1e30f, "lstm: x_abs_bound must be 0 (measure) or a finite positive bound");
  RNNT_CHECK_ARG(!d->row_idx || (d->n_rows >= 1 && d->n_rows <= (int64_t)d->T * d->B), "lstm: row_idx needs 1 <= n_rows <= T*B (got %d)", d->n_rows);
  *w = carve_lstm(d->workspace, d->T, d->B, d->I, d->H, d->D, *pl);
  RNNT_CHECK_ARG(d->workspace && d->workspace_bytes >= w->total, "lstm: workspace too small (%zu < %zu)",
                 d->workspace_bytes, w->total);
  RNNT_CHECK_ARG((reinterpret_cast<uintptr_t>(d->gates) & 15) == 0 && (reinterpret_cast<uintptr_t>(d->y) & 15) == 0 &&
                     (reinterpret_cast<uintptr_t>(d->cst) & 15) == 0 && (reinterpret_cast<uintptr_t>(d->aux) & 15) == 0 &&
                     (reinterpret_cast<uintptr_t>(d->workspace) & 255) == 0,
                 "lstm: gates/y/cst must be 16-byte aligned, workspace 256-byte aligned");
  return RNNT_OK;
}

void fill_kernel_args(const rnnt_lstm_desc* d, const Plan& pl, const LstmWs& w, LstmK* k) {
  k->T = d->T; k->B = d->B; k->H = d->H; k->D = d->D;
  k->Hs = pl.Hs; k->NC = pl.NC; k->Bp = pl.Bp; k->LDW = pl.LDW;
  k->lens = d->lens; k->gates = d->gates; k->cst = d->cst; k->y = d->y;
  k->ydrop = d->dropout_p > 0.f ? d->y_drop : nullptr;
  k->keep_scale = d->dropout_p > 0.f ? 1.f / (1.f - d->dropout_p) : 1.f;
  k->drop_thresh = (unsigned)((double)d->dropout_p * 4294967296.0);
  k->seed = d->dropout_seed;
  k->w_hh[0] = d->w_hh[0]; k->w_hh[1] = d->D > 1 ? d->w_hh[1] : d->w_hh[0];
  k->hx = w.hx; k->status = d->status ? d->status : w.flags; k->flags = w.flags + 16;
  k->dy = nullptr;
  k->cell = d->cell;
  k->b_hh[0] = d->b_hh[0]; k->b_hh[1] = d->D > 1 ? d->b_hh[1] : d->b_hh[0];
  k->aux = d->aux;
  k->G = 1; k->Bg = d->B; k->Kp = d->H; k->NGL = d->D;
  k->dbp = w.dbp; k->dbhp = w.dbp + w.dbp_half;
  k->dbg = getenv("RNNT_LSTM_DBG") ? w.dbg : nullptr;
  k->xcc = w.flags + 16 + w.nflags;
  k->allow_local = getenv("RNNT_LSTM_NO_XCD_LOCAL") ? 0 : 1;
  k->hw_math = getenv("RNNT_LSTM_EXACT_MATH") ? 0 : 1;
  k->pause = 0;
  k->gbound = 0;
  k->colmax = k->colmax_h = nullptr;
  k->rowmax = nullptr;
}

bool shape_takes_row_idx(int T, int B, int I, int H, int D, int cell, int cus) {
  Plan2 p2;
  return use_hp(T, B, I, H, D) && I >= 32 && T > 1 && make_plan3(B, H, D, cus, true, &p2) && lstm5_supported(T, B, H, D, cell);
}
bool shape_takes_f16(int T, int B, int I, int H, int D, int cell, int cus) {
  Plan2 pf, pb;
  return use_hp(T, B, I, H, D) && make_plan3(B, H, D, cus, false, &pf) && make_plan3(B, H, D, cus, true, &pb) &&
         lstm5_supported(T, B, H, D, cell);
}
bool ragged_plan(const rnnt_lstm_desc* d, const LstmWs& w, int cus) {
  return d->row_idx && d->n_rows > 0 && d->n_rows < (int64_t)d->T * d->B && w.hp && d->x_sb == d->I && d->x_st == (int64_t)d->B * d->I &&
         shape_takes_row_idx(d->T, d->B, d->I, d->H, d->D, d->cell, cus);
}

}
}

using namespace rnnt;

extern "C" int32_t rnnt_hip_lstm_max_batch(int32_t H, int32_t D, int32_t cell) {
  int cus = device_cus();
  if (cus <= 0) cus = 256;
  int best = 0;
  for (int B = 64; B >= 1; --B) {
    Plan2 p2;
    Plan p1;
    if (make_plan3(B, H, D, cus, true, &p2) || make_plan2(B, H, D, cus, &p2) || (cell == RNNT_CELL_LSTM && make_plan(B, H, D, cus, &p1))) { best = B; break; }
  }
  return best;
}

static int recurrence_xcds(int T, int B, int H, int D, int cell, int cus) {
  Plan2 p2;
  if (!make_plan3(B, H, D, cus, true, &p2) || !lstm5_supported(T, B, H, D, cell)) return 8;
  const int NG = D * p2.G;
  return (NG <= 4 && p2.NC <= 32 && !getenv("RNNT_LSTM_NO_XCD_STRIDE")) ? NG : 8;
}

extern "C" int32_t rnnt_hip_lstm_takes_row_idx(int32_t T, int32_t B, int32_t I, int32_t H, int32_t D, int32_t cell) {
  int cus = device_cus();
  if (cus <= 0) cus = 256;
  if (T < 1 || B < 1 || I < 1 || H < 4 || D < 1 || D > 2) return 0;
  return shape_takes_row_idx(T, B, I, H, D, cell, cus) ? 1 : 0;
}

extern "C" int32_t rnnt_hip_lstm_takes_f16(int32_t T, int32_t B, int32_t I, int32_t H, int32_t D, int32_t cell) {
  int cus = device_cus();
  if (cus <= 0) cus = 256;
  if (T < 1 || B < 1 || I < 1 || H < 4 || D < 1 || D > 2) return 0;
  return shape_takes_f16(T, B, I, H, D, cell, cus) ? 1 : 0;
}

extern "C" int32_t rnnt_hip_lstm_free_xcds(int32_t T, int32_t B, int32_t H, int32_t D, int32_t cell) {
  int cus = device_cus();
  if (cus <= 0) cus = 256;
  if (T < 1 || B < 1 || H < 4 || D < 1 || D > 2) return 0;
  return 8 - recurrence_xcds(T, B, H, D, cell, cus);
}

extern "C" size_t rnnt_hip_lstm_workspace_bytes(int32_t T, int32_t B, int32_t I, int32_t H, int32_t D) {
  Plan pl;
  int cus = device_cus();
  if (cus <= 0) cus = 256;
  if (T < 1 || I < 1 || !make_plan(B, H, D, cus, &pl)) return 0;
  return carve_lstm(nullptr, T, B, I, H, D, pl).total;
}

static int lstm_fwd_impl(const rnnt_lstm_desc* d, uint32_t precision, void* stream) {
  Plan pl;
  LstmWs w;
  if (int rc = check_desc(d, &pl, &w)) return rc;
  hipStream_t s = (hipStream_t)stream;
  const int H = d->H, D = d->D, I = d->I;
  const bool f16 = precision == RNNT_PRECISION_F16 && shape_takes_f16(d->T, d->B, I, H, D, d->cell, device_cus());
  const unsigned hpf = f16 ? RNNT_GEMM_HP_F16 : 0u;
  const int ngate = d->cell == RNNT_CELL_LSTM ? 4 : (d->cell == RNNT_CELL_GRU ? 3 : 1);
  {
    const long per = (long)4 * H * I;
    hipLaunchKernelGGL(permute_w_kernel, dim3((unsigned)ceil_div(per, 256), D), dim3(256), 0, s, d->w_ih[0],
                       D > 1 ? d->w_ih[1] : d->w_ih[0], H, I, ngate, w.wp);
    RNNT_CHECK_LAUNCH();
    hipLaunchKernelGGL(permute_bias_kernel, dim3((unsigned)ceil_div(4 * H, 256), D), dim3(256), 0, s, d->b_ih[0], d->b_hh[0],
                       D > 1 ? d->b_ih[1] : d->b_ih[0], D > 1 ? d->b_hh[1] : d->b_hh[0], H, ngate,
                       d->cell == RNNT_CELL_GRU ? 1 : 0, w.bp);
    RNNT_CHECK_LAUNCH();
  }
  const bool x_plain = d->x_sb == I && d->x_st == (int64_t)d->B * I;
  const bool ragged = ragged_plan(d, w, device_cus());
  if (w.hp && x_plain && I >= 32) {
    const int64_t M = (int64_t)d->T * d->B, N4 = (int64_t)D * 4 * H;
    const int64_t Mv = ragged ? d->n_rows : M;
    const int* ridx = ragged ? d->row_idx : nullptr;
    uint32_t* ax = w.hp_amax, *aw = w.hp_amax + M;
    if (int rc = hp_split(d->x, Mv, I, I, ax, w.hp_x, s, ridx)) return rc;
    if (int rc = hp_split(w.wp, N4, I, I, aw, w.hp_w, s)) return rc;
    if (int rc = hp_gemm(w.hp_x, ax, w.hp_w, aw, Mv, N4, I, d->gates, 1, N4, 0, w.bp, hpf, nullptr, 0, s, ridx, M, ridx)) return rc;
  } else {
    rnnt_gemm_desc g = {};
    g.M = (int64_t)d->T * d->B; g.N = (int64_t)D * 4 * H; g.K = I;
    g.A = d->x; g.a_div = d->B; g.a_so = d->x_st; g.a_si = d->x_sb; g.a_sk = 1; g.a_mc = 0;
    g.B = w.wp; g.b_sn = I; g.b_sk = 1;
    g.C = d->gates; g.c_div = 1; g.c_so = g.N; g.c_si = 0;
    g.bias = w.bp;
    if (int rc = rnnt_hip_gemm_f32(&g, s)) return rc;
  }
  RNNT_CHECK_HIP(hipMemsetAsync(w.flags, 0, (size_t)(reinterpret_cast<char*>(w.hx) - reinterpret_cast<char*>(w.flags)) + w.hx_bytes, s));
  LstmK k;
  fill_kernel_args(d, pl, w, &k);
  k.gbound = ragged ? 1 : 0;
  int rc = RNNT_OK;
  Plan2 p2;
  const int cus = device_cus();
  auto adopt = [&](const Plan2& q) {
    k.NC = q.NC; k.Hs = q.HS; k.G = q.G; k.Bg = q.Bg; k.Kp = q.Kp;
  };
  if (make_plan3(d->B, d->H, d->D, cus, false, &p2)) {
    adopt(p2);
    const int nks = p2.Kp / 128, c = cell_form(d->cell);
    if (lstm5_supported(d->T, d->B, d->H, d->D, d->cell)) {
      rc = lstm5_fwd_launch(k, p2, d->cell, s, f16);
    } else if (p2.MB == 5) {
      const size_t lds5 = p2.lds_fwd + 8 * 1 * 3 * 3 * 1024;
      rc = dispatch<0, 1, 2>(c, "lstm_fwd3 cell", [&](auto C) {
        return launch_persistent2(lstm_fwd3_kernel<3, C, 8, 5, 1>, k, p2, lds5, s, "lstm_fwd3", 512);
      });
    } else if (nks == 4) {
      const size_t lds = (size_t)8 * 4 * 64 * 16 + 16;
      rc = dispatch<0, 1, 2>(c, "lstm_fwd3 cell", [&](auto C) {
        return launch_persistent2(lstm_fwd3_kernel<2, C, 8>, k, p2, lds, s, "lstm_fwd3", 512);
      });
    } else if (nks <= 3) {
      rc = dispatch<1, 2, 3>(nks, "lstm_fwd3 k-steps", [&](auto N) {
        return dispatch<0, 1, 2>(c, "lstm_fwd3 cell", [&](auto C) {
          return launch_persistent2(lstm_fwd3_kernel<N, C>, k, p2, p2.lds_fwd, s, "lstm_fwd3");
        });
      });
    } else {
      rc = dispatch<3, 4>(p2.Kp / (32 * 8), "lstm_fwd3 k-steps", [&](auto N) {
        const size_t lds8 = p2.lds_fwd + 8 * 1 * N * 3 * 1024;
        return dispatch<0, 1, 2>(c, "lstm_fwd3 cell", [&](auto C) {
          return launch_persistent2(lstm_fwd3_kernel<N, C, 8, 4, 1>, k, p2, lds8, s, "lstm_fwd3", 512);
        });
      });
    }
  } else if (make_plan2(d->B, d->H, d->D, cus, &p2)) {
    adopt(p2);
    rc = dispatch<4, 8, 16>(p2.HS, "lstm_fwd2 HS", [&](auto HS) {
      return dispatch<1, 2, 4>(p2.BQ, "lstm_fwd2 BQ", [&](auto BQ) {
        return dispatch<0, 1, 2>(cell_form(d->cell), "lstm_fwd2 cell", [&](auto C) {
          return launch_persistent2(lstm_fwd2_kernel<HS, BQ, C>, k, p2, p2.lds_fwd, s, "lstm_fwd2");
        });
      });
    });
  } else if (d->cell == RNNT_CELL_LSTM) {
    rc = dispatch<1, 2, 4>(pl.MT, "lstm_fwd MT", [&](auto MT) {
      return dispatch<1, 2, 4>(pl.NT, "lstm_fwd NT", [&](auto NT) {
        return launch_persistent(lstm_fwd_kernel<MT, NT>, k, pl, pl.lds_fwd, s, "lstm_fwd");
      });
    });
  } else {
    set_error("rnn: GRU / Elman cells need the grouped decomposition (B/G <= 16 rows per group); B=%d H=%d does not fit", d->B, d->H);
    rc = RNNT_ERR_UNSUPPORTED;
  }
  return rc;
}

extern "C" int rnnt_hip_lstm_fwd(const rnnt_lstm_desc* d, void* stream) { return lstm_fwd_impl(d, RNNT_PRECISION_FP32, stream); }

extern "C" int rnnt_hip_lstm_fwd_ex(const rnnt_lstm_desc* d, uint32_t precision, void* stream) {
  RNNT_CHECK_ARG(precision == RNNT_PRECISION_FP32 || precision == RNNT_PRECISION_F16, "lstm_fwd_ex: precision must be 0 (fp32) or 1 (f16), got %u",
                 precision);
  return lstm_fwd_impl(d, precision, stream);
}

static int lstm_bwd_impl(const rnnt_lstm_bwd_desc* bd, uint32_t precision, void* stream) {
  RNNT_CHECK_ARG(bd != nullptr, "lstm_bwd: null descriptor");
  const rnnt_lstm_desc* d = &bd->f;
  Plan pl;
  LstmWs w;
  if (int rc = check_desc(d, &pl, &w)) return rc;
  RNNT_CHECK_ARG(bd->dy, "lstm_bwd: null dy");
  const int T = d->T, B = d->B, H = d->H, D = d->D, I = d->I;
  const bool f16 = precision == RNNT_PRECISION_F16 && shape_takes_f16(T, B, I, H, D, d->cell, device_cus());
  const unsigned hpf = f16 ? RNNT_GEMM_HP_F16 : 0u;
  const bool gru = d->cell == RNNT_CELL_GRU;
  const int ngate = d->cell == RNNT_CELL_LSTM ? 4 : (gru ? 3 : 1);
  RNNT_CHECK_ARG(!gru || d->aux, "lstm_bwd: GRU needs the aux buffer (T,B,D*4H)");
  for (int k = 0; k < D; ++k) RNNT_CHECK_ARG(!gru || bd->db_hh[k], "lstm_bwd: GRU needs db_hh");
  const int acc = bd->accumulate ? 1 : 0;
  float* twin0 = gru ? nullptr : bd->db_hh[0];
  float* twin1 = gru ? nullptr : (D > 1 ? bd->db_hh[1] : bd->db_hh[0]);
  if (twin0 == bd->db[0]) twin0 = nullptr;
  if (twin1 == (D > 1 ? bd->db[1] : bd->db[0])) twin1 = nullptr;
  const float* ghid = gru ? d->aux : d->gates;
  RNNT_CHECK_ARG(d->x_sb == I && d->x_st == (int64_t)B * I, "lstm_bwd: x must be time-major contiguous (T,B,I)");
  for (int k = 0; k < D; ++k) RNNT_CHECK_ARG(bd->dw_ih[k] && bd->dw_hh[k] && bd->db[k], "lstm_bwd: null gradient output");
  hipStream_t s = (hipStream_t)stream;
  RNNT_CHECK_ARG(bd->phase >= RNNT_LSTM_BWD_ALL && bd->phase <= RNNT_LSTM_BWD_WEIGHTS, "lstm_bwd: phase must be 0, 1 or 2");
  const bool do_recur = bd->phase != RNNT_LSTM_BWD_WEIGHTS, do_weights = bd->phase != RNNT_LSTM_BWD_RECUR;

  if (do_recur)
    RNNT_CHECK_HIP(hipMemsetAsync(w.flags, 0, (size_t)(reinterpret_cast<char*>(w.hx) - reinterpret_cast<char*>(w.flags)) + w.hx_bytes, s));
  LstmK k;
  fill_kernel_args(d, pl, w, &k);
  k.dy = bd->dy;
  int rc = RNNT_OK;
  Plan2 p2;
  const int cus = device_cus();
  const bool ragged = ragged_plan(d, w, cus);
  const int* ridx = ragged ? d->row_idx : nullptr;
  k.gbound = ragged ? 1 : 0;
  auto adopt = [&](const Plan2& q) {
    k.NC = q.NC; k.Hs = q.HS; k.G = q.G; k.Bg = q.Bg; k.Kp = q.Kp;
  };
  bool fused_db = false, colmax_done = false, rowmax_done = false;
  int db_rows = 0;
  unsigned xcd_skip = 0;
  if (make_plan3(d->B, d->H, d->D, cus, true, &p2)) {
    adopt(p2);
    fused_db = true;
    db_rows = p2.G * 4 * p2.BQ;
    const int c = cell_form(d->cell);
    if (lstm5_supported(d->T, d->B, d->H, d->D, d->cell)) {
      if (w.hp) {
        const int64_t Mr = (int64_t)T * B, N4r = (int64_t)D * 4 * H;
        k.colmax = w.hp_amax + Mr + N4r + Mr;
        k.colmax_h = w.hp_amax + 2 * Mr + 2 * N4r + 2 * I + (int64_t)D * H;
        unsigned* fill_from = k.colmax;
        if (!gru && I >= 128 && bd->dx && !getenv("RNNT_GEMM_HP_NO_FUSED_SPLIT")) {
          k.rowmax = w.hp_amax + Mr + N4r;
          fill_from = k.rowmax;
          rowmax_done = true;
        }
        if (do_recur)
          RNNT_CHECK_HIP(hipMemsetAsync(fill_from, 0, (size_t)(k.colmax_h + N4r - fill_from) * 4, s));
        colmax_done = true;
      }
      if (do_recur) rc = lstm5_bwd_launch(k, p2, d->cell, s, f16);
      if (bd->beside_recurrence) {
        const int used = recurrence_xcds(T, B, H, D, d->cell, cus);
        if (used <= 4 && cus == 256) xcd_skip = (1u << used) - 1u;
      }
    } else if (!do_recur) {
    } else if (p2.MB == 5) {
      rc = dispatch<1, 2, 4>(p2.BQ, "lstm_bwd4 BQ", [&](auto BQ) {
        return dispatch<0, 1, 2>(c, "lstm_bwd4 cell", [&](auto C) {
          return launch_persistent2(lstm_bwd4_kernel<6, BQ, C, 8, 5, 1>, k, p2, p2.lds_bwd + 8 * 1 * 3 * 3 * 1024, s, "lstm_bwd4", 512);
        });
      });
    } else if (p2.Kp <= 512) {
      rc = dispatch<2, 4, 6, 8>(p2.Kp / (16 * 4), "lstm_bwd4 output blocks", [&](auto NOB) {
        return dispatch<1, 2, 4>(p2.BQ, "lstm_bwd4 BQ", [&](auto BQ) {
          return dispatch<0, 1, 2>(c, "lstm_bwd4 cell", [&](auto C) {
            return launch_persistent2(lstm_bwd4_kernel<NOB, BQ, C>, k, p2, p2.lds_bwd, s, "lstm_bwd4");
          });
        });
      });
    } else {
      rc = dispatch<6, 8>(p2.Kp / (16 * 8), "lstm_bwd4 output blocks", [&](auto NOB) {
        return dispatch<1, 2, 4>(p2.BQ, "lstm_bwd4 BQ", [&](auto BQ) {
          return dispatch<0, 1, 2>(c, "lstm_bwd4 cell", [&](auto C) {
            return launch_persistent2(lstm_bwd4_kernel<NOB, BQ, C, 8, 4, 2>, k, p2, p2.lds_bwd + 8 * 2 * 2 * 3 * 1024, s, "lstm_bwd4", 512);
          });
        });
      });
    }
  } else if (make_plan2(d->B, d->H, d->D, cus, &p2)) {
    adopt(p2);
    if (do_recur)
      rc = dispatch<4, 8, 16>(p2.HS, "lstm_bwd2 HS", [&](auto HS) {
        return dispatch<1, 2, 4>(p2.BQ, "lstm_bwd2 BQ", [&](auto BQ) {
          return dispatch<0, 1, 2>(cell_form(d->cell), "lstm_bwd2 cell", [&](auto C) {
            return launch_persistent2(lstm_bwd2_kernel<HS, BQ, C>, k, p2, p2.lds_bwd, s, "lstm_bwd2");
          });
        });
      });
  } else if (d->cell == RNNT_CELL_LSTM) {
    if (do_recur)
      rc = dispatch<1, 2, 4>(pl.MT, "lstm_bwd MT", [&](auto MT) {
        return dispatch<1, 2, 4>(pl.NT, "lstm_bwd NT", [&](auto NT) {
          return launch_persistent(lstm_bwd_kernel<MT, NT>, k, pl, pl.lds_bwd, s, "lstm_bwd");
        });
      });
  } else {
    set_error("rnn: GRU / Elman cells need the grouped decomposition; B=%d H=%d does not fit", d->B, d->H);
    rc = RNNT_ERR_UNSUPPORTED;
  }
  if (rc) return rc;

  const int64_t M = (int64_t)T * B, N4 = (int64_t)D * 4 * H;
  const int64_t Mv = ragged ? d->n_rows : M;
  const bool hp_in = w.hp && I >= 128;
  uint32_t* a_dgr = w.hp ? w.hp_amax + M + N4 : nullptr;
  uint32_t* a_dgc = w.hp ? a_dgr + M : nullptr;
  uint32_t* a_w = w.hp ? a_dgc + N4 : nullptr;
  uint32_t* a_x = w.hp ? a_w + I : nullptr;
  uint32_t* a_y = w.hp ? a_x + I : nullptr;
  if (w.hp) {
    const bool both = rowmax_done && colmax_done && hp_in && bd->dx;
    if (do_recur && hp_in && bd->dx) {
      if (both) rc = hp_split_both(d->gates, Mv, N4, N4, a_dgr, a_dgc, w.hp_dg, w.hp_dgt, s, ridx);
      else rc = hp_split(d->gates, Mv, N4, N4, a_dgr, w.hp_dg, s, ridx);
      if (rc) return rc;
    }
    if (do_weights && !colmax_done)
      if ((rc = hp_colmax(d->gates, M, N4, N4, a_dgc, s))) return rc;
    if (do_weights && !both)
      if ((rc = hp_split_t(d->gates, N4, Mv, N4, M, 0, a_dgc, w.hp_dgt, s, ridx))) return rc;
  }
  if (do_recur && bd->dx) {
    const long per = (long)4 * H * I;
    hipLaunchKernelGGL(permute_w_kernel, dim3((unsigned)ceil_div(per, 256), D), dim3(256), 0, s, d->w_ih[0],
                       D > 1 ? d->w_ih[1] : d->w_ih[0], H, I, ngate, w.wp);
    RNNT_CHECK_LAUNCH();
    if (hp_in) {
      if ((rc = hp_colmax(w.wp, N4, I, I, a_w, s))) return rc;
      if ((rc = hp_split_t(w.wp, I, N4, I, N4, 0, a_w, w.hp_w, s))) return rc;
      if ((rc = hp_gemm(w.hp_dg, a_dgr, w.hp_w, a_w, Mv, I, N4, bd->dx, 1, I, 0, nullptr, hpf, nullptr, 0, s, ridx, M, ridx))) return rc;
    } else {
      rnnt_gemm_desc g = {};
      g.M = M; g.N = I; g.K = N4;
      g.A = d->gates; g.a_div = 1; g.a_so = N4; g.a_si = 0; g.a_sk = 1; g.a_mc = 0;
      g.B = w.wp; g.b_sn = 1; g.b_sk = I;
      g.C = bd->dx; g.c_div = 1; g.c_so = I; g.c_si = 0;
      if ((rc = rnnt_hip_gemm_f32(&g, s))) return rc;
    }
    if (ragged) {
      const long nrow = (long)T * B;
      hipLaunchKernelGGL(zero_padded_rows_kernel, dim3((unsigned)(ceil_div(nrow, 4) < 2048 ? ceil_div(nrow, 4) : 2048)), dim3(256), 0, s, bd->dx, d->lens, T, B, I);
      RNNT_CHECK_LAUNCH();
    }
  }
  if (!do_weights) return RNNT_OK;
  const bool grouped = w.hp && hp_in && T > 1 && !gru && D <= 2 && (xcd_skip != 0u || getenv("RNNT_GEMM_HP_GROUP")) && !getenv("RNNT_GEMM_HP_NO_GROUP");
  {
    const bool x_plain = d->x_sb == I && d->x_st == (int64_t)B * I;
    if (hp_in || (w.hp && I >= 32 && x_plain && !getenv("RNNT_GEMM_HP_NO_NARROW"))) {
      if (d->x_abs_bound > 0.f) {
        uint32_t bits;
        memcpy(&bits, &d->x_abs_bound, 4);
        RNNT_CHECK_HIP(hipMemsetD32Async((hipDeviceptr_t)a_x, (int)bits, (size_t)I, s));
      } else if ((rc = hp_colmax(d->x, M, I, I, a_x, s))) return rc;
      if ((rc = hp_split_t(d->x, I, Mv, I, M, 0, a_x, w.hp_x, s, ridx))) return rc;
      if (!grouped)
        if ((rc = hp_gemm(w.hp_dgt, a_dgc, w.hp_x, a_x, N4, I, Mv, w.wp, 1, I, 0, nullptr, hpf, w.scratch, w.scratch_bytes, s))) return rc;
    } else {
      rnnt_gemm_desc g = {};
      g.M = N4; g.N = I; g.K = M;
      g.A = d->gates; g.a_mc = 1; g.a_sk = N4; g.a_div = 1;
      g.B = d->x; g.b_sn = 1; g.b_sk = I;
      g.C = w.wp; g.c_div = 1; g.c_so = I; g.c_si = 0;
      g.workspace = w.scratch; g.workspace_bytes = w.scratch_bytes;
      if ((rc = rnnt_hip_gemm_f32(&g, s))) return rc;
    }
    if (!grouped) {
      const long per = (long)4 * H * I;
      hipLaunchKernelGGL(unpermute_w_kernel, dim3((unsigned)ceil_div(per, 256), D), dim3(256), 0, s, w.wp, H, I, per, ngate,
                         bd->dw_ih[0], D > 1 ? bd->dw_ih[1] : bd->dw_ih[0], acc);
      RNNT_CHECK_LAUNCH();
    }
  }
  if (w.hp && T > 1) {
    if (d->cell != RNNT_CELL_RNN_RELU) {
      RNNT_CHECK_HIP(hipMemsetD32Async((hipDeviceptr_t)a_y, 0x3f800000, (size_t)D * H, s));
    } else if ((rc = hp_colmax(d->y, M, (int64_t)D * H, (int64_t)D * H, a_y, s))) return rc;
    if (gru) {
      if (colmax_done) a_dgc = a_y + (int64_t)D * H;
      else if ((rc = hp_colmax(ghid, M, N4, N4, a_dgc, s))) return rc;
      if ((rc = hp_split_t(ghid, N4, Mv, N4, M, 0, a_dgc, w.hp_dgt, s, ridx))) return rc;
    }
    HpProblem pr[HP_GROUP_MAX];
    int npr = 0;
    if (grouped) pr[npr++] = HpProblem{w.hp_dgt, a_dgc, w.hp_x, a_x, N4, I, Mv, w.wp, I, hpf};
    for (int dir = 0; dir < D; ++dir) {
      char* yt = w.hp_yt + (size_t)dir * hp_plane_bytes(H, M);
      if ((rc = hp_split_t(d->y + (int64_t)dir * H, H, Mv, (int64_t)D * H, M, dir == 0 ? -B : B, a_y + (int64_t)dir * H, yt, s, ridx))) return rc;
      const char* ag = w.hp_dgt + (size_t)dir * 4 * H * (size_t)ceil_div(Mv, 32) * 128;
      if (grouped) {
        pr[npr++] = HpProblem{ag, a_dgc + (int64_t)dir * 4 * H, yt, a_y + (int64_t)dir * H, 4 * H, H, Mv, w.dwhh + (int64_t)dir * 4 * H * H, H, hpf};
        continue;
      }
      if ((rc = hp_gemm(ag, a_dgc + (int64_t)dir * 4 * H, yt, a_y + (int64_t)dir * H, 4 * H, H, Mv, w.dwhh + (int64_t)dir * 4 * H * H, 1, H, 0,
                        nullptr, hpf, w.scratch, w.scratch_bytes, s)))
        return rc;
    }
    if (grouped) {
      if ((rc = hp_gemm_grouped(pr, npr, xcd_skip, reinterpret_cast<unsigned*>(w.scratch), (char*)w.scratch + HPQ_HEADER_BYTES,
                                w.scratch_bytes - HPQ_HEADER_BYTES, s, k.status)))
        return rc;
      const long per = (long)4 * H * I;
      hipLaunchKernelGGL(unpermute_w_kernel, dim3((unsigned)ceil_div(per, 256), D), dim3(256), 0, s, w.wp, H, I, per, ngate,
                         bd->dw_ih[0], D > 1 ? bd->dw_ih[1] : bd->dw_ih[0], acc);
      RNNT_CHECK_LAUNCH();
    }
  } else
  for (int dir = 0; dir < D; ++dir) {
    rnnt_gemm_desc g = {};
    g.M = 4 * H; g.N = H; g.K = (int64_t)(T - 1) * B;
    const int64_t shift_g = dir == 0 ? (int64_t)B * N4 : 0;
    const int64_t shift_y = dir == 0 ? 0 : (int64_t)B * D * H;
    g.A = ghid + shift_g + (int64_t)dir * 4 * H; g.a_mc = 1; g.a_sk = N4; g.a_div = 1;
    g.B = d->y + shift_y + (int64_t)dir * H; g.b_sn = 1; g.b_sk = (int64_t)D * H;
    g.C = w.dwhh + (int64_t)dir * 4 * H * H; g.c_div = 1; g.c_so = H; g.c_si = 0;
    g.workspace = w.scratch; g.workspace_bytes = w.scratch_bytes;
    if (g.K > 0) {
      if ((rc = rnnt_hip_gemm_f32(&g, s))) return rc;
    } else {
      RNNT_CHECK_HIP(hipMemsetAsync(g.C, 0, (size_t)4 * H * H * 4, s));
    }
  }
  {
    const long per = (long)4 * H * H;
    hipLaunchKernelGGL(unpermute_w_kernel, dim3((unsigned)ceil_div(per, 256), D), dim3(256), 0, s, w.dwhh, H, H, per, ngate,
                       bd->dw_hh[0], D > 1 ? bd->dw_hh[1] : bd->dw_hh[0], acc);
    RNNT_CHECK_LAUNCH();
  }
  if (fused_db) {
    hipLaunchKernelGGL(db_reduce_kernel, dim3((unsigned)ceil_div(4 * H, 256), D), dim3(256), 0, s, k.dbp, db_rows, H, ngate, bd->db[0],
                       D > 1 ? bd->db[1] : bd->db[0], acc, twin0, twin1);
    RNNT_CHECK_LAUNCH();
    if (gru) {
      hipLaunchKernelGGL(db_reduce_kernel, dim3((unsigned)ceil_div(4 * H, 256), D), dim3(256), 0, s, k.dbhp, db_rows, H, ngate, bd->db_hh[0],
                         D > 1 ? bd->db_hh[1] : bd->db_hh[0], acc);
      RNNT_CHECK_LAUNCH();
    }
  } else {
    if ((rc = launch_colsum(d->gates, (long)M, (long)N4, (long)N4, w.bp, w.scratch, w.scratch_bytes, s))) return rc;
    hipLaunchKernelGGL(unpermute_w_kernel, dim3((unsigned)ceil_div(4 * H, 256), D), dim3(256), 0, s, w.bp, H, 1, (long)4 * H, ngate,
                       bd->db[0], D > 1 ? bd->db[1] : bd->db[0], acc, twin0, twin1);
    RNNT_CHECK_LAUNCH();
    if (gru) {
      if ((rc = launch_colsum(ghid, (long)M, (long)N4, (long)N4, w.bp, w.scratch, w.scratch_bytes, s))) return rc;
      hipLaunchKernelGGL(unpermute_w_kernel, dim3((unsigned)ceil_div(4 * H, 256), D), dim3(256), 0, s, w.bp, H, 1, (long)4 * H, ngate,
                         bd->db_hh[0], D > 1 ? bd->db_hh[1] : bd->db_hh[0], acc);
      RNNT_CHECK_LAUNCH();
    }
  }
  return RNNT_OK;
}

extern "C" int rnnt_hip_lstm_bwd(const rnnt_lstm_bwd_desc* bd, void* stream) { return lstm_bwd_impl(bd, RNNT_PRECISION_FP32, stream); }

extern "C" int rnnt_hip_lstm_bwd_ex(const rnnt_lstm_bwd_desc* bd, uint32_t precision, void* stream) {
  RNNT_CHECK_ARG(precision == RNNT_PRECISION_FP32 || precision == RNNT_PRECISION_F16, "lstm_bwd_ex: precision must be 0 (fp32) or 1 (f16), got %u",
                 precision);
  return lstm_bwd_impl(bd, precision, stream);
}

extern "C" int rnnt_hip_lstm_check(const void* workspace, void* stream) {
  RNNT_CHECK_ARG(workspace != nullptr, "lstm_check: null workspace");
  unsigned st = 0;
  RNNT_CHECK_HIP(hipMemcpyAsync(&st, workspace, sizeof(st), hipMemcpyDeviceToHost, (hipStream_t)stream));
  RNNT_CHECK_HIP(hipStreamSynchronize((hipStream_t)stream));
  if (st != 0) {
    set_error("persistent LSTM kernel abandoned an inter-workgroup wait (status %u)", st);
    return RNNT_ERR_TIMEOUT;
  }
  return RNNT_OK;
}

extern "C" int rnnt_hip_lstm_debug_read(const void* workspace, int32_t T, int32_t B, int32_t I, int32_t H, int32_t D,
                                        uint64_t* out, int32_t nwg, void* stream) {
  Plan pl;
  int cus = device_cus();
  RNNT_CHECK_ARG(workspace && out && nwg >= 1 && nwg <= 512, "lstm_debug_read: bad arguments");
  RNNT_CHECK_ARG(make_plan(B, H, D, cus, &pl), "lstm_debug_read: unsupported shape");
  const LstmWs w = carve_lstm(const_cast<void*>(workspace), T, B, I, H, D, pl);
  RNNT_CHECK_HIP(hipMemcpyAsync(out, w.dbg, (size_t)nwg * 8 * 8, hipMemcpyDeviceToHost, (hipStream_t)stream));
  RNNT_CHECK_HIP(hipStreamSynchronize((hipStream_t)stream));
  return RNNT_OK;
}

extern "C" size_t rnnt_hip_colsum_workspace_bytes(int64_t M, int64_t N) {
  if (M < 0 || N < 1) return 0;
  return (size_t)colsum_chunks((long)M, (long)N) * (size_t)N * 4;
}

extern "C" int rnnt_hip_colsum_f32(const float* X, int64_t M, int64_t N, int64_t ld, float* out, void* workspace,
                                   size_t workspace_bytes, void* stream) {
  RNNT_CHECK_ARG(X && out && M >= 0 && N >= 1 && ld >= N, "colsum: bad arguments");
  return launch_colsum(X, (long)M, (long)N, (long)ld, out, workspace, workspace_bytes, (hipStream_t)stream);
}
extern "C" int rnnt_hip_colsum_f32_acc(const float* X, int64_t M, int64_t N, int64_t ld, float* out, void* workspace,
                                       size_t workspace_bytes, void* stream) {
  RNNT_CHECK_ARG(X && out && M >= 0 && N >= 1 && ld >= N, "colsum: bad arguments");
  return launch_colsum(X, (long)M, (long)N, (long)ld, out, workspace, workspace_bytes, (hipStream_t)stream, 1);
}

extern "C" int rnnt_hip_embedding_fwd(const float* W, const int64_t* idx, int64_t M, int32_t H, int32_t V, float* out,
                                      void* stream) {
  RNNT_CHECK_ARG(W && idx && out && M >= 0 && H >= 1 && V >= 1, "embedding_fwd: bad arguments");
  if (M == 0) return RNNT_OK;
  const long blocks = ceil_div(M * H, 256);
  hipLaunchKernelGGL(embedding_fwd_kernel, dim3((unsigned)(blocks < 4096 ? blocks : 4096)), dim3(256), 0, (hipStream_t)stream, W,
                     (const long*)idx, (long)M, H, V, out);
  RNNT_CHECK_LAUNCH();
  return RNNT_OK;
}

static int embedding_bwd_impl(const float* dE, const int64_t* idx, int64_t M, int32_t H, int32_t V, int64_t padding_idx,
                              float* dW, int accumulate, void* stream) {
  RNNT_CHECK_ARG(dE && idx && dW && M >= 0 && H >= 1 && V >= 1, "embedding_bwd: bad arguments");
  hipLaunchKernelGGL(embedding_bwd_kernel, dim3(V), dim3(256), 0, (hipStream_t)stream, dE, (const long*)idx, (long)M, H, V,
                     (long)padding_idx, dW, accumulate);
  RNNT_CHECK_LAUNCH();
  return RNNT_OK;
}
extern "C" int rnnt_hip_embedding_bwd(const float* dE, const int64_t* idx, int64_t M, int32_t H, int32_t V,
                                      int64_t padding_idx, float* dW, void* stream) {
  return embedding_bwd_impl(dE, idx, M, H, V, padding_idx, dW, 0, stream);
}
extern "C" int rnnt_hip_embedding_bwd_acc(const float* dE, const int64_t* idx, int64_t M, int32_t H, int32_t V,
                                          int64_t padding_idx, float* dW, void* stream) {
  return embedding_bwd_impl(dE, idx, M, H, V, padding_idx, dW, 1, stream);
}
```

Baseline: 1290.

## Fuse gate permute/unpermute into HP split and GEMM epilogues in LSTM backward

```diff
diff --git a/include/rnnt_hip.h b/include/rnnt_hip.h
--- a/include/rnnt_hip.h
+++ b/include/rnnt_hip.h
@@ -70,6 +70,12 @@
                       void* planes, uint32_t* amax, int32_t amax_given, void* stream);
 int rnnt_hip_hp_split_both(const float* x, int64_t M, int64_t C, int64_t ld, const uint32_t* rowmax, const uint32_t* colmax,
                            void* planes_rm, void* planes_t, void* stream);
+int rnnt_hip_hp_split_gates(const float* w0, const float* w1, int32_t H, int64_t I, int32_t D, int32_t ngate, int32_t transpose,
+                            void* planes, uint32_t* amax, const float* b_ih0, const float* b_hh0, const float* b_ih1,
+                            const float* b_hh1, int32_t gru, float* bias_out, void* stream);
+int rnnt_hip_gemm_hp_gates(const void* A, const uint32_t* a_amax, const void* B, const uint32_t* b_amax, int64_t M, int64_t N, int64_t K,
+                           float* dw0, float* dw1, int32_t H, int32_t ngate, uint32_t flags, void* workspace, size_t workspace_bytes,
+                           void* stream);
 size_t rnnt_hip_gemm_hp_workspace_bytes(int64_t M, int64_t N, int64_t K);
 int rnnt_hip_gemm_hp(const void* A, const uint32_t* a_amax, const void* B, const uint32_t* b_amax, int64_t M, int64_t N, int64_t K,
                      float* C, int64_t ldc, const float* bias, uint32_t flags, void* workspace, size_t workspace_bytes,
@@ -146,6 +152,9 @@
 int rnnt_hip_lstm_bwd(const rnnt_lstm_bwd_desc* d, void* stream);
 int rnnt_hip_lstm_bwd_ex(const rnnt_lstm_bwd_desc* d, uint32_t precision, void* stream);
 int rnnt_hip_lstm_check(const void* workspace, void* stream);
+int rnnt_hip_lstm_gate_permute(const float* w0, const float* w1, int32_t H, int64_t I, int32_t D, int32_t ngate, float* out, void* stream);
+int rnnt_hip_lstm_gate_unpermute(const float* in, int32_t H, int64_t I, int32_t D, int32_t ngate, float* o0, float* o1, int32_t accumulate,
+                                 void* stream);
 int rnnt_hip_lstm_debug_read(const void* workspace, int32_t T, int32_t B, int32_t I, int32_t H, int32_t D,
                              uint64_t* out, int32_t nwg, void* stream);
 
diff --git a/rnntransducer_amd/_lib.py b/rnntransducer_amd/_lib.py
--- a/rnntransducer_amd/_lib.py
+++ b/rnntransducer_amd/_lib.py
@@ -135,6 +135,12 @@
     "rnnt_hip_gemm_hp": (C.c_int, [C.c_void_p, C.c_void_p, C.c_void_p, C.c_void_p, c_i64, c_i64, c_i64, C.c_void_p, c_i64, C.c_void_p,
                                   C.c_uint32, C.c_void_p, C.c_size_t, C.c_void_p]),
     "rnnt_hip_hp_split_both": (C.c_int, [C.c_void_p, c_i64, c_i64, c_i64, C.c_void_p, C.c_void_p, C.c_void_p, C.c_void_p, C.c_void_p]),
+    "rnnt_hip_hp_split_gates": (C.c_int, [C.c_void_p, C.c_void_p, c_i32, c_i64, c_i32, c_i32, c_i32, C.c_void_p, C.c_void_p, C.c_void_p,
+                                         C.c_void_p, C.c_void_p, C.c_void_p, c_i32, C.c_void_p, C.c_void_p]),
+    "rnnt_hip_gemm_hp_gates": (C.c_int, [C.c_void_p, C.c_void_p, C.c_void_p, C.c_void_p, c_i64, c_i64, c_i64, C.c_void_p, C.c_void_p, c_i32,
+                                        c_i32, C.c_uint32, C.c_void_p, C.c_size_t, C.c_void_p]),
+    "rnnt_hip_lstm_gate_permute": (C.c_int, [C.c_void_p, C.c_void_p, c_i32, c_i64, c_i32, c_i32, C.c_void_p, C.c_void_p]),
+    "rnnt_hip_lstm_gate_unpermute": (C.c_int, [C.c_void_p, c_i32, c_i64, c_i32, c_i32, C.c_void_p, C.c_void_p, c_i32, C.c_void_p]),
     "rnnt_hip_gemm_hp_grouped_workspace_bytes": (C.c_size_t, [C.POINTER(HpProblem), c_i32]),
     "rnnt_hip_gemm_hp_grouped": (C.c_int, [C.POINTER(HpProblem), c_i32, C.c_uint32, C.c_void_p, C.c_size_t, C.c_void_p]),
     "rnnt_hip_lstm_workspace_bytes": (C.c_size_t, [c_i32] * 5),
diff --git a/rnntransducer_amd/csrc/common.hpp b/rnntransducer_amd/csrc/common.hpp
--- a/rnntransducer_amd/csrc/common.hpp
+++ b/rnntransducer_amd/csrc/common.hpp
@@ -48,14 +48,19 @@
 size_t hp_plane_bytes(int64_t rows, int64_t K);
 int hp_colmax(const float* x, int64_t rows, int64_t C, int64_t ld, uint32_t* amax, hipStream_t s);
 int hp_split(const float* x, int64_t rows, int64_t K, int64_t ld, uint32_t* amax, void* planes, hipStream_t s, const int* rowidx = nullptr);
-int hp_split_t(const float* x, int64_t R, int64_t K, int64_t ld, int64_t Ksrc, int64_t shift, const uint32_t* amax, void* planes,
-               hipStream_t s, const int* kidx = nullptr);
+struct HpSplitDirs { int n; int64_t x_dz, amax_dz, planes_dz, shift_dz; };
+int hp_split_t(const float* x, int64_t R, int64_t K, int64_t ld, int64_t Ksrc, int64_t shift, uint32_t* amax, void* planes,
+               hipStream_t s, const int* kidx = nullptr, uint32_t amax_const = 0, const HpSplitDirs* dirs = nullptr);
+int hp_split_gates(const float* w0, const float* w1, int H, int64_t I, int D, int ngate, uint32_t* amax, void* planes, const float* const* b_ih,
+                   const float* const* b_hh, int gru, float* bp, hipStream_t s);
+int hp_split_t_gates(const float* w0, const float* w1, int H, int64_t I, int D, int ngate, uint32_t* amax, bool zeroed, void* planes, hipStream_t s);
+struct HpOutMap { float* C1; int H, ngate; };
 int hp_split_both(const float* x, int64_t M, int64_t C, int64_t ld, const uint32_t* rowmax, const uint32_t* colmax, void* planes_rm,
                   void* planes_t, hipStream_t s, const int* rowidx = nullptr);
 size_t hp_gemm_workspace_bytes(int64_t M, int64_t N, int64_t K);
 int hp_gemm(const void* A, const uint32_t* a_amax, const void* B, const uint32_t* b_amax, int64_t M, int64_t N, int64_t K, float* C,
             int64_t c_div, int64_t c_so, int64_t c_si, const float* bias, unsigned flags, void* workspace, size_t workspace_bytes,
-            hipStream_t s, const int* a_rowidx = nullptr, int64_t a_plane_rows = 0, const int* c_rowidx = nullptr);
+            hipStream_t s, const int* a_rowidx = nullptr, int64_t a_plane_rows = 0, const int* c_rowidx = nullptr, const HpOutMap* omap = nullptr);
 struct HpProblem {
   const void* A; const uint32_t* a_amax; const void* B; const uint32_t* b_amax;
   int64_t M, N, K;
diff --git a/rnntransducer_amd/csrc/gemm_hp.hip b/rnntransducer_amd/csrc/gemm_hp.hip
--- a/rnntransducer_amd/csrc/gemm_hp.hip
+++ b/rnntransducer_amd/csrc/gemm_hp.hip
@@ -25,10 +25,11 @@
   return __uint_as_float((unsigned)(eb - 14) << 23);
 }
 
-__global__ void __launch_bounds__(256) hp_colmax_kernel(const float* __restrict__ x, long rows, int C, long ld, long rows_per_chunk,
-                                                        unsigned* __restrict__ out) {
+__global__ void __launch_bounds__(256) hp_colmax_kernel(const float* __restrict__ x0, const float* __restrict__ x1, long rows, int C, long ld,
+                                                        long rows_per_chunk, unsigned* __restrict__ out) {
   const int c = blockIdx.x * 256 + threadIdx.x;
   if (c >= C) return;
+  const float* x = blockIdx.z ? x1 : x0;
   const long r0 = (long)blockIdx.y * rows_per_chunk, r1 = min(rows, r0 + rows_per_chunk);
   unsigned m = 0;
   for (long r = r0; r < r1; ++r) m = max(m, __float_as_uint(x[r * ld + c]) & 0x7fffffffu);
@@ -92,22 +93,104 @@
   }
 }
 
+struct HpGateMap {
+  const float* w1;
+  int H, ngate;
+};
+__device__ __forceinline__ const float* hp_gate_row(const float* w0, const HpGateMap& gm, int r, long ld) {
+  const int per = 4 * gm.H, dir = r / per, rr = r - dir * per, g = rr & 3;
+  if (g >= gm.ngate) return nullptr;
+  return (dir ? gm.w1 : w0) + (long)(g * gm.H + (rr >> 2)) * ld;
+}
+
+struct HpGateBias { const float* bi[2]; const float* bh[2]; float* bp; int gru; };
+__global__ void __launch_bounds__(256) hp_split_gates_kernel(const float* __restrict__ x, const HpGateMap gm, long rows, int K, long ld,
+                                                             unsigned* __restrict__ amax, char* __restrict__ out, const HpGateBias gb) {
+  const int Kp = (K + 31) & ~31, cpr = Kp >> 3;
+  const int lane = threadIdx.x & 63;
+  const bool vec = (ld & 3) == 0 && ((reinterpret_cast<uintptr_t>(x) | reinterpret_cast<uintptr_t>(gm.w1)) & 15) == 0;
+  for (long r = (long)blockIdx.x * 4 + (threadIdx.x >> 6); r < rows; r += (long)gridDim.x * 4) {
+    const float* row = hp_gate_row(x, gm, (int)r, ld);
+    unsigned m = 0;
+    if (row)
+      for (int c = lane; c < cpr; c += 64) {
+        const int k = 8 * c;
+        if (vec && k + 7 < K) {
+          const u32x4 a = *reinterpret_cast<const u32x4*>(row + k), b = *reinterpret_cast<const u32x4*>(row + k + 4);
+#pragma unroll
+          for (int e = 0; e < 4; ++e) m = max(m, max(a[e] & 0x7fffffffu, b[e] & 0x7fffffffu));
+        } else {
+#pragma unroll
+          for (int e = 0; e < 8; ++e)
+            if (k + e < K) m = max(m, __float_as_uint(row[k + e]) & 0x7fffffffu);
+        }
+      }
+#pragma unroll
+    for (int o = 32; o > 0; o >>= 1) m = max(m, (unsigned)__shfl_xor((int)m, o));
+    if (lane == 0) {
+      amax[r] = m;
+      if (gb.bp) {
+        const int per = 4 * gm.H, dir = (int)r / per, rr = (int)r - dir * per, g = rr & 3, src = g * gm.H + (rr >> 2);
+        float v = 0.f;
+        if (g < gm.ngate) {
+          const float bi = gb.bi[dir][src], bh = gb.bh[dir][src];
+          v = (gb.gru && g == 2) ? bi : bi + bh;
+        }
+        gb.bp[r] = v;
+      }
+    }
+    const float scale = hp_scale_from_amax(m);
+    for (int c = lane; c < cpr; c += 64) {
+      const int k = 8 * c;
+      float v[8];
+      if (!row) {
+#pragma unroll
+        for (int e = 0; e < 8; ++e) v[e] = 0.f;
+      } else if (vec && k + 7 < K) {
+        const f32x4 a = *reinterpret_cast<const f32x4*>(row + k), b = *reinterpret_cast<const f32x4*>(row + k + 4);
+        v[0] = a[0]; v[1] = a[1]; v[2] = a[2]; v[3] = a[3]; v[4] = b[0]; v[5] = b[1]; v[6] = b[2]; v[7] = b[3];
+      } else {
+#pragma unroll
+        for (int e = 0; e < 8; ++e) v[e] = (k + e < K) ? row[k + e] : 0.f;
+      }
+      u32x4 hi, lo;
+      hp_split8(v, scale, hi, lo);
+      char* dst = out + (r * (Kp >> 5) + (c >> 2)) * 128 + 16 * (c & 3);
+      *reinterpret_cast<u32x4*>(dst) = hi;
+      *reinterpret_cast<u32x4*>(dst + 64) = lo;
+    }
+  }
+}
+
+struct HpSplitZ { long x_dz, amax_dz, out_dz; int shift_dz; };
+template <bool GATES>
 __global__ void __launch_bounds__(256) hp_split_t_kernel(const float* __restrict__ x, int R, int K, long ld, int Ksrc, int shift,
-                                                         const unsigned* __restrict__ amax, char* __restrict__ out,
-                                                         const int* __restrict__ kidx) {
+                                                         unsigned* __restrict__ amax, char* __restrict__ out,
+                                                         const int* __restrict__ kidx, const HpSplitZ zs, const unsigned amax_const,
+                                                         const HpGateMap gm) {
   __shared__ float tile[32][257];
   const int kb = blockIdx.x, r0 = blockIdx.y * 256;
   const int tid = threadIdx.x;
-  const bool vec = (ld & 3) == 0 && (reinterpret_cast<uintptr_t>(x) & 15) == 0;
+  {
+    const int z = blockIdx.z;
+    x += z * zs.x_dz; amax += z * zs.amax_dz; out += z * zs.out_dz; shift += z * zs.shift_dz;
+  }
+  const bool vec = (ld & 3) == 0 && ((reinterpret_cast<uintptr_t>(x) | (GATES ? reinterpret_cast<uintptr_t>(gm.w1) : 0)) & 15) == 0;
 #pragma unroll
   for (int q = 0; q < 8; ++q) {
     const int kk = 4 * q + (tid >> 6);
     const int kdst = kb * 32 + kk;
-    const int ksrc = (kidx ? (kdst < K ? kidx[kdst] : 0) : kdst) + shift;
     const int c = 4 * (tid & 63);
     f32x4 v = {0.f, 0.f, 0.f, 0.f};
-    if (kdst < K && ksrc >= 0 && ksrc < Ksrc) {
-      const float* src = x + (long)ksrc * ld + r0 + c;
+    const float* srow = nullptr;
+    if constexpr (GATES) {
+      if (kdst < K) srow = hp_gate_row(x, gm, kdst, ld);
+    } else {
+      const int ksrc = (kidx ? (kdst < K ? kidx[kdst] : 0) : kdst) + shift;
+      if (kdst < K && ksrc >= 0 && ksrc < Ksrc) srow = x + (long)ksrc * ld;
+    }
+    if (srow) {
+      const float* src = srow + r0 + c;
       if (vec && r0 + c + 3 < R) {
         v = *reinterpret_cast<const f32x4*>(src);
       } else {
@@ -129,7 +212,9 @@
 #pragma unroll
       for (int e = 0; e < 8; ++e) v[e] = tile[8 * ch + e][rl];
       u32x4 hi, lo;
-      hp_split8(v, hp_scale_from_amax(amax[r0 + rl]), hi, lo);
+      const unsigned am = amax_const ? amax_const : amax[r0 + rl];
+      if (amax_const && kb == 0 && ch == 0) amax[r0 + rl] = am;
+      hp_split8(v, hp_scale_from_amax(am), hi, lo);
       char* dst = out + ((long)(r0 + rl) * Kp32 + kb) * 128 + 16 * ch;
       *reinterpret_cast<u32x4*>(dst) = hi;
       *reinterpret_cast<u32x4*>(dst + 64) = lo;
@@ -204,7 +289,13 @@
   int group_m;
   const int* a_rowidx;
   const int* c_rowidx;
+  float* C1; int map_H, map_ngate;
 };
+__device__ __forceinline__ float* hp_mapped_row(const HpGemmK& p, int m, bool* stored) {
+  const int per = 4 * p.map_H, dir = m / per, rr = m - dir * per, g = rr & 3;
+  *stored = g < p.map_ngate;
+  return (dir ? p.C1 : p.C) + (long)((*stored ? g : 0) * p.map_H + (rr >> 2)) * p.c_so;
+}
 
 __device__ __forceinline__ int hp_xcd_remap(int bid, int n) {
   const int q = n / 8, r = n % 8, xcd = bid % 8;
@@ -331,11 +422,17 @@
 #pragma unroll
     for (int reg = 0; reg < 4; ++reg) {
       const int m = m0 + wr * 128 + i * 16 + 4 * (lane >> 4) + reg;
-      const bool mok = m < p.M;
+      bool mok = m < p.M;
       const int mc = mok ? m : 0;
       const float sa = hp_inv_scale_from_amax(p.a_amax[p.a_rowidx ? p.a_rowidx[mc] : mc]);
       const int mo = p.c_rowidx ? p.c_rowidx[mc] : mc;
-      float* crow = mode == 0 ? slab + (long)mc * p.N : p.C + (long)(mo / p.c_div) * p.c_so + (long)(mo % p.c_div) * p.c_si;
+      float* crow;
+      if (mode == 0) crow = slab + (long)mc * p.N;
+      else if (p.map_H > 0) {
+        bool stored;
+        crow = hp_mapped_row(p, mc, &stored);
+        mok = mok && stored;
+      } else crow = p.C + (long)(mo / p.c_div) * p.c_so + (long)(mo % p.c_div) * p.c_si;
       float old[4] = {0.f, 0.f, 0.f, 0.f};
       if (mode == 2) {
 #pragma unroll
@@ -428,10 +525,17 @@
     float s = 0.f;
     for (int z = 0; z < p.splits; ++z) s += p.slab[(long)z * total + i];
     if (p.bias) s += p.bias[n];
-    const int mo = p.c_rowidx ? p.c_rowidx[m] : m;
-    const long off = (long)(mo / p.c_div) * p.c_so + (long)(mo % p.c_div) * p.c_si + n;
-    if (p.flags & RNNT_GEMM_ACCUM) s += p.C[off];
-    p.C[off] = s;
+    float* dst;
+    if (p.map_H > 0) {
+      bool stored;
+      dst = hp_mapped_row(p, m, &stored) + n;
+      if (!stored) continue;
+    } else {
+      const int mo = p.c_rowidx ? p.c_rowidx[m] : m;
+      dst = p.C + (long)(mo / p.c_div) * p.c_so + (long)(mo % p.c_div) * p.c_si + n;
+    }
+    if (p.flags & RNNT_GEMM_ACCUM) s += *dst;
+    *dst = s;
   }
 }
 
@@ -447,7 +551,7 @@
   if (chunks < 1) chunks = 1;
   const long rpc = ceil_div(rows, chunks);
   ProfScope prof(RNNT_K_HP_SPLIT, 4.0 * (double)rows * (double)C, s);
-  hipLaunchKernelGGL(hp_colmax_kernel, dim3((unsigned)ceil_div(C, 256), (unsigned)ceil_div(rows, rpc)), dim3(256), 0, s, x, (long)rows, (int)C,
+  hipLaunchKernelGGL(hp_colmax_kernel, dim3((unsigned)ceil_div(C, 256), (unsigned)ceil_div(rows, rpc)), dim3(256), 0, s, x, x, (long)rows, (int)C,
                      (long)ld, rpc, amax);
   RNNT_CHECK_LAUNCH();
   return RNNT_OK;
@@ -463,12 +567,51 @@
   return RNNT_OK;
 }
 
-int hp_split_t(const float* x, int64_t R, int64_t K, int64_t ld, int64_t Ksrc, int64_t shift, const uint32_t* amax, void* planes,
-               hipStream_t s, const int* kidx) {
+int hp_split_t(const float* x, int64_t R, int64_t K, int64_t ld, int64_t Ksrc, int64_t shift, uint32_t* amax, void* planes,
+               hipStream_t s, const int* kidx, uint32_t amax_const, const HpSplitDirs* dirs) {
   if (R == 0 || K == 0) return RNNT_OK;
-  ProfScope prof(RNNT_K_HP_SPLIT, 8.0 * (double)R * (double)K, s);
-  hipLaunchKernelGGL(hp_split_t_kernel, dim3((unsigned)ceil_div(K, 32), (unsigned)ceil_div(R, 256)), dim3(256), 0, s, x, (int)R, (int)K, (long)ld,
-                     (int)Ksrc, (int)shift, amax, (char*)planes, kidx);
+  const int nz = dirs ? dirs->n : 1;
+  HpSplitZ zs = {0, 0, 0, 0};
+  if (dirs) zs = HpSplitZ{(long)dirs->x_dz, (long)dirs->amax_dz, (long)dirs->planes_dz, (int)dirs->shift_dz};
+  ProfScope prof(RNNT_K_HP_SPLIT, 8.0 * (double)R * (double)K * nz, s);
+  hipLaunchKernelGGL(hp_split_t_kernel<false>, dim3((unsigned)ceil_div(K, 32), (unsigned)ceil_div(R, 256), (unsigned)nz), dim3(256), 0, s, x, (int)R,
+                     (int)K, (long)ld, (int)Ksrc, (int)shift, amax, (char*)planes, kidx, zs, (unsigned)amax_const, HpGateMap{nullptr, 0, 0});
+  RNNT_CHECK_LAUNCH();
+  return RNNT_OK;
+}
+
+int hp_split_gates(const float* w0, const float* w1, int H, int64_t I, int D, int ngate, uint32_t* amax, void* planes, const float* const* b_ih,
+                   const float* const* b_hh, int gru, float* bp, hipStream_t s) {
+  const long rows = (long)D * 4 * H;
+  if (rows == 0) return RNNT_OK;
+  HpGateBias gb = {};
+  if (bp) {
+    gb.bi[0] = b_ih[0]; gb.bh[0] = b_hh[0];
+    gb.bi[1] = D > 1 ? b_ih[1] : b_ih[0]; gb.bh[1] = D > 1 ? b_hh[1] : b_hh[0];
+    gb.bp = bp; gb.gru = gru;
+  }
+  const long blocks = ceil_div(rows, 4);
+  ProfScope prof(RNNT_K_HP_SPLIT, 8.0 * (double)rows * (double)I, s);
+  hipLaunchKernelGGL(hp_split_gates_kernel, dim3((unsigned)(blocks < 8192 ? blocks : 8192)), dim3(256), 0, s, w0, HpGateMap{D > 1 ? w1 : w0, H, ngate},
+                     rows, (int)I, (long)I, amax, (char*)planes, gb);
+  RNNT_CHECK_LAUNCH();
+  return RNNT_OK;
+}
+
+int hp_split_t_gates(const float* w0, const float* w1, int H, int64_t I, int D, int ngate, uint32_t* amax, bool zeroed, void* planes, hipStream_t s) {
+  const long rows = (long)ngate * H, N4 = (long)D * 4 * H;
+  if (!zeroed) RNNT_CHECK_HIP(hipMemsetAsync(amax, 0, (size_t)I * 4, s));
+  if (N4 == 0 || I == 0) return RNNT_OK;
+  long chunks = ceil_div(2048, ceil_div(I, 256) * D);
+  if (chunks > ceil_div(rows, 64)) chunks = ceil_div(rows, 64);
+  if (chunks < 1) chunks = 1;
+  const long rpc = ceil_div(rows, chunks);
+  ProfScope prof(RNNT_K_HP_SPLIT, 12.0 * (double)N4 * (double)I, s);
+  hipLaunchKernelGGL(hp_colmax_kernel, dim3((unsigned)ceil_div(I, 256), (unsigned)ceil_div(rows, rpc), (unsigned)D), dim3(256), 0, s, w0,
+                     D > 1 ? w1 : w0, rows, (int)I, (long)I, rpc, amax);
+  RNNT_CHECK_LAUNCH();
+  hipLaunchKernelGGL(hp_split_t_kernel<true>, dim3((unsigned)ceil_div(N4, 32), (unsigned)ceil_div(I, 256), 1), dim3(256), 0, s, w0, (int)I, (int)N4,
+                     (long)I, (int)N4, 0, amax, (char*)planes, (const int*)nullptr, HpSplitZ{0, 0, 0, 0}, 0u, HpGateMap{D > 1 ? w1 : w0, H, ngate});
   RNNT_CHECK_LAUNCH();
   return RNNT_OK;
 }
@@ -495,8 +638,11 @@
 
 int hp_gemm(const void* A, const uint32_t* a_amax, const void* B, const uint32_t* b_amax, int64_t M, int64_t N, int64_t K, float* C,
             int64_t c_div, int64_t c_so, int64_t c_si, const float* bias, unsigned flags, void* workspace, size_t workspace_bytes,
-            hipStream_t s, const int* a_rowidx, int64_t a_plane_rows, const int* c_rowidx) {
+            hipStream_t s, const int* a_rowidx, int64_t a_plane_rows, const int* c_rowidx, const HpOutMap* omap) {
   RNNT_CHECK_ARG(A && B && C && a_amax && b_amax, "gemm_hp: null operand");
+  RNNT_CHECK_ARG(!omap || (omap->H >= 1 && omap->ngate >= 1 && omap->ngate <= 4 && M % (4 * (int64_t)omap->H) == 0 && M / (4 * (int64_t)omap->H) <= 2 &&
+                           (omap->C1 || M == 4 * (int64_t)omap->H) && !c_rowidx && !bias && c_div == 1),
+                 "gemm_hp: a gate-mapped output is 4H or 2 x 4H rows, plain row stride, no bias / row scatter");
   RNNT_CHECK_ARG(!a_rowidx || a_plane_rows >= M, "gemm_hp: a gathered A operand needs the row count of its planes");
   RNNT_CHECK_ARG(M >= 1 && N >= 1 && K >= 1 && M < (1ll << 31) && N < (1ll << 31) && K < (1ll << 31), "gemm_hp: bad dims");
   RNNT_CHECK_ARG(c_div >= 1, "gemm_hp: c_div must be >= 1");
@@ -511,6 +657,7 @@
   k.C = C; k.c_div = (int)(c_div > 0x7fffffff ? 0x7fffffff : c_div); k.c_so = c_so; k.c_si = c_si;
   k.bias = bias; k.flags = flags;
   k.a_rowidx = a_rowidx; k.c_rowidx = c_rowidx;
+  k.C1 = omap ? omap->C1 : nullptr; k.map_H = omap ? omap->H : 0; k.map_ngate = omap ? omap->ngate : 0;
   const bool f16 = (flags & RNNT_GEMM_HP_F16) != 0u;
   k.tiles_m = (int)ceil_div(M, HP_BM); k.tiles_n = (int)ceil_div(N, HP_BN);
   const int tiles = k.tiles_m * k.tiles_n;
@@ -584,6 +731,7 @@
     k.C = a.C; k.c_div = 1; k.c_so = a.ldc; k.c_si = 0;
     k.bias = nullptr; k.flags = a.flags;
     k.a_rowidx = k.c_rowidx = nullptr;
+    k.C1 = nullptr; k.map_H = k.map_ngate = 0;
     k.tiles_m = (int)ceil_div(a.M, HP_BM); k.tiles_n = (int)ceil_div(a.N, HP_BN);
     total_kt += (long)k.tiles_m * k.tiles_n * k.nkt;
     flops += 2.0 * (double)a.M * (double)a.N * (double)a.K;
@@ -696,3 +844,22 @@
   RNNT_CHECK_ARG(((reinterpret_cast<uintptr_t>(planes_rm) | reinterpret_cast<uintptr_t>(planes_t)) & 127) == 0, "hp_split_both: planes must be 128-byte aligned");
   return hp_split_both(x, M, C, ld, rowmax, colmax, planes_rm, planes_t, (hipStream_t)stream);
 }
+
+extern "C" int rnnt_hip_hp_split_gates(const float* w0, const float* w1, int32_t H, int64_t I, int32_t D, int32_t ngate, int32_t transpose,
+                                       void* planes, uint32_t* amax, const float* b_ih0, const float* b_hh0, const float* b_ih1,
+                                       const float* b_hh1, int32_t gru, float* bias_out, void* stream) {
+  RNNT_CHECK_ARG(w0 && planes && amax && H >= 1 && I >= 1 && (D == 1 || (D == 2 && w1)) && ngate >= 1 && ngate <= 4, "hp_split_gates: bad arguments");
+  RNNT_CHECK_ARG((reinterpret_cast<uintptr_t>(planes) & 127) == 0, "hp_split_gates: planes must be 128-byte aligned");
+  RNNT_CHECK_ARG(!bias_out || (!transpose && b_ih0 && b_hh0 && (D == 1 || (b_ih1 && b_hh1))), "hp_split_gates: bias_out needs b_ih / b_hh (row-major form only)");
+  if (transpose) return hp_split_t_gates(w0, w1, H, I, D, ngate, amax, false, planes, (hipStream_t)stream);
+  const float* bi[2] = {b_ih0, b_ih1};
+  const float* bh[2] = {b_hh0, b_hh1};
+  return hp_split_gates(w0, w1, H, I, D, ngate, amax, planes, bi, bh, gru, bias_out, (hipStream_t)stream);
+}
+
+extern "C" int rnnt_hip_gemm_hp_gates(const void* A, const uint32_t* a_amax, const void* B, const uint32_t* b_amax, int64_t M, int64_t N,
+                                      int64_t K, float* dw0, float* dw1, int32_t H, int32_t ngate, uint32_t flags, void* workspace,
+                                      size_t workspace_bytes, void* stream) {
+  const HpOutMap om = {dw1, H, ngate};
+  return hp_gemm(A, a_amax, B, b_amax, M, N, K, dw0, 1, N, 0, nullptr, flags, workspace, workspace_bytes, (hipStream_t)stream, nullptr, 0, nullptr, &om);
+}
diff --git a/rnntransducer_amd/csrc/lstm.hip b/rnntransducer_amd/csrc/lstm.hip
--- a/rnntransducer_amd/csrc/lstm.hip
+++ b/rnntransducer_amd/csrc/lstm.hip
@@ -1613,7 +1613,9 @@
   const bool f16 = precision == RNNT_PRECISION_F16 && shape_takes_f16(d->T, d->B, I, H, D, d->cell, device_cus());
   const unsigned hpf = f16 ? RNNT_GEMM_HP_F16 : 0u;
   const int ngate = d->cell == RNNT_CELL_LSTM ? 4 : (d->cell == RNNT_CELL_GRU ? 3 : 1);
-  {
+  const bool x_plain = d->x_sb == I && d->x_st == (int64_t)d->B * I;
+  const bool hp_proj = w.hp && x_plain && I >= 32;
+  if (!hp_proj) {
     const long per = (long)4 * H * I;
     hipLaunchKernelGGL(permute_w_kernel, dim3((unsigned)ceil_div(per, 256), D), dim3(256), 0, s, d->w_ih[0],
                        D > 1 ? d->w_ih[1] : d->w_ih[0], H, I, ngate, w.wp);
@@ -1623,15 +1625,14 @@
                        d->cell == RNNT_CELL_GRU ? 1 : 0, w.bp);
     RNNT_CHECK_LAUNCH();
   }
-  const bool x_plain = d->x_sb == I && d->x_st == (int64_t)d->B * I;
   const bool ragged = ragged_plan(d, w, device_cus());
-  if (w.hp && x_plain && I >= 32) {
+  if (hp_proj) {
     const int64_t M = (int64_t)d->T * d->B, N4 = (int64_t)D * 4 * H;
     const int64_t Mv = ragged ? d->n_rows : M;
     const int* ridx = ragged ? d->row_idx : nullptr;
     uint32_t* ax = w.hp_amax, *aw = w.hp_amax + M;
     if (int rc = hp_split(d->x, Mv, I, I, ax, w.hp_x, s, ridx)) return rc;
-    if (int rc = hp_split(w.wp, N4, I, I, aw, w.hp_w, s)) return rc;
+    if (int rc = hp_split_gates(d->w_ih[0], d->w_ih[1], H, I, D, ngate, aw, w.hp_w, d->b_ih, d->b_hh, d->cell == RNNT_CELL_GRU ? 1 : 0, w.bp, s)) return rc;
     if (int rc = hp_gemm(w.hp_x, ax, w.hp_w, aw, Mv, N4, I, d->gates, 1, N4, 0, w.bp, hpf, nullptr, 0, s, ridx, M, ridx)) return rc;
   } else {
     rnnt_gemm_desc g = {};
@@ -1752,6 +1753,7 @@
     k.NC = q.NC; k.Hs = q.HS; k.G = q.G; k.Bg = q.Bg; k.Kp = q.Kp;
   };
   bool fused_db = false, colmax_done = false, rowmax_done = false;
+  const unsigned* cleared_from = nullptr, *cleared_to = nullptr;
   int db_rows = 0;
   unsigned xcd_skip = 0;
   if (make_plan3(d->B, d->H, d->D, cus, true, &p2)) {
@@ -1770,8 +1772,10 @@
           fill_from = k.rowmax;
           rowmax_done = true;
         }
-        if (do_recur)
+        if (do_recur) {
           RNNT_CHECK_HIP(hipMemsetAsync(fill_from, 0, (size_t)(k.colmax_h + N4r - fill_from) * 4, s));
+          cleared_from = fill_from; cleared_to = k.colmax_h + N4r;
+        }
         colmax_done = true;
       }
       if (do_recur) rc = lstm5_bwd_launch(k, p2, d->cell, s, f16);
@@ -1847,15 +1851,15 @@
       if ((rc = hp_split_t(d->gates, N4, Mv, N4, M, 0, a_dgc, w.hp_dgt, s, ridx))) return rc;
   }
   if (do_recur && bd->dx) {
-    const long per = (long)4 * H * I;
-    hipLaunchKernelGGL(permute_w_kernel, dim3((unsigned)ceil_div(per, 256), D), dim3(256), 0, s, d->w_ih[0],
-                       D > 1 ? d->w_ih[1] : d->w_ih[0], H, I, ngate, w.wp);
-    RNNT_CHECK_LAUNCH();
     if (hp_in) {
-      if ((rc = hp_colmax(w.wp, N4, I, I, a_w, s))) return rc;
-      if ((rc = hp_split_t(w.wp, I, N4, I, N4, 0, a_w, w.hp_w, s))) return rc;
+      const bool a_w_cleared = cleared_from && a_w >= cleared_from && a_w + I <= cleared_to;
+      if ((rc = hp_split_t_gates(d->w_ih[0], d->w_ih[1], H, I, D, ngate, a_w, a_w_cleared, w.hp_w, s))) return rc;
       if ((rc = hp_gemm(w.hp_dg, a_dgr, w.hp_w, a_w, Mv, I, N4, bd->dx, 1, I, 0, nullptr, hpf, nullptr, 0, s, ridx, M, ridx))) return rc;
     } else {
+      const long per = (long)4 * H * I;
+      hipLaunchKernelGGL(permute_w_kernel, dim3((unsigned)ceil_div(per, 256), D), dim3(256), 0, s, d->w_ih[0],
+                         D > 1 ? d->w_ih[1] : d->w_ih[0], H, I, ngate, w.wp);
+      RNNT_CHECK_LAUNCH();
       rnnt_gemm_desc g = {};
       g.M = M; g.N = I; g.K = N4;
       g.A = d->gates; g.a_div = 1; g.a_so = N4; g.a_si = 0; g.a_sk = 1; g.a_mc = 0;
@@ -1871,17 +1875,22 @@
   }
   if (!do_weights) return RNNT_OK;
   const bool grouped = w.hp && hp_in && T > 1 && !gru && D <= 2 && (xcd_skip != 0u || getenv("RNNT_GEMM_HP_GROUP")) && !getenv("RNNT_GEMM_HP_NO_GROUP");
+  const unsigned accf = acc ? RNNT_GEMM_ACCUM : 0u;
   {
     const bool x_plain = d->x_sb == I && d->x_st == (int64_t)B * I;
+    bool direct = false;
     if (hp_in || (w.hp && I >= 32 && x_plain && !getenv("RNNT_GEMM_HP_NO_NARROW"))) {
-      if (d->x_abs_bound > 0.f) {
-        uint32_t bits;
-        memcpy(&bits, &d->x_abs_bound, 4);
-        RNNT_CHECK_HIP(hipMemsetD32Async((hipDeviceptr_t)a_x, (int)bits, (size_t)I, s));
-      } else if ((rc = hp_colmax(d->x, M, I, I, a_x, s))) return rc;
-      if ((rc = hp_split_t(d->x, I, Mv, I, M, 0, a_x, w.hp_x, s, ridx))) return rc;
-      if (!grouped)
-        if ((rc = hp_gemm(w.hp_dgt, a_dgc, w.hp_x, a_x, N4, I, Mv, w.wp, 1, I, 0, nullptr, hpf, w.scratch, w.scratch_bytes, s))) return rc;
+      uint32_t xbits = 0;
+      if (d->x_abs_bound > 0.f) memcpy(&xbits, &d->x_abs_bound, 4);
+      else if ((rc = hp_colmax(d->x, M, I, I, a_x, s))) return rc;
+      if ((rc = hp_split_t(d->x, I, Mv, I, M, 0, a_x, w.hp_x, s, ridx, xbits))) return rc;
+      if (!grouped) {
+        const HpOutMap om = {D > 1 ? bd->dw_ih[1] : bd->dw_ih[0], H, ngate};
+        if ((rc = hp_gemm(w.hp_dgt, a_dgc, w.hp_x, a_x, N4, I, Mv, bd->dw_ih[0], 1, I, 0, nullptr, hpf | accf, w.scratch, w.scratch_bytes, s, nullptr, 0,
+                          nullptr, &om)))
+          return rc;
+        direct = true;
+      }
     } else {
       rnnt_gemm_desc g = {};
       g.M = N4; g.N = I; g.K = M;
@@ -1891,37 +1900,45 @@
       g.workspace = w.scratch; g.workspace_bytes = w.scratch_bytes;
       if ((rc = rnnt_hip_gemm_f32(&g, s))) return rc;
     }
-    if (!grouped) {
+    if (!grouped && !direct) {
       const long per = (long)4 * H * I;
       hipLaunchKernelGGL(unpermute_w_kernel, dim3((unsigned)ceil_div(per, 256), D), dim3(256), 0, s, w.wp, H, I, per, ngate,
                          bd->dw_ih[0], D > 1 ? bd->dw_ih[1] : bd->dw_ih[0], acc);
       RNNT_CHECK_LAUNCH();
     }
   }
+  bool dwhh_direct = false;
   if (w.hp && T > 1) {
-    if (d->cell != RNNT_CELL_RNN_RELU) {
-      RNNT_CHECK_HIP(hipMemsetD32Async((hipDeviceptr_t)a_y, 0x3f800000, (size_t)D * H, s));
-    } else if ((rc = hp_colmax(d->y, M, (int64_t)D * H, (int64_t)D * H, a_y, s))) return rc;
+    uint32_t ybits = 0x3f800000u;
+    if (d->cell == RNNT_CELL_RNN_RELU) {
+      ybits = 0;
+      if ((rc = hp_colmax(d->y, M, (int64_t)D * H, (int64_t)D * H, a_y, s))) return rc;
+    }
     if (gru) {
       if (colmax_done) a_dgc = a_y + (int64_t)D * H;
       else if ((rc = hp_colmax(ghid, M, N4, N4, a_dgc, s))) return rc;
       if ((rc = hp_split_t(ghid, N4, Mv, N4, M, 0, a_dgc, w.hp_dgt, s, ridx))) return rc;
+    }
+    {
+      const HpSplitDirs dirs = {D, H, H, (int64_t)hp_plane_bytes(H, M), 2 * (int64_t)B};
+      if ((rc = hp_split_t(d->y, H, Mv, (int64_t)D * H, M, -B, a_y, w.hp_yt, s, ridx, ybits, &dirs))) return rc;
     }
     HpProblem pr[HP_GROUP_MAX];
     int npr = 0;
     if (grouped) pr[npr++] = HpProblem{w.hp_dgt, a_dgc, w.hp_x, a_x, N4, I, Mv, w.wp, I, hpf};
     for (int dir = 0; dir < D; ++dir) {
       char* yt = w.hp_yt + (size_t)dir * hp_plane_bytes(H, M);
-      if ((rc = hp_split_t(d->y + (int64_t)dir * H, H, Mv, (int64_t)D * H, M, dir == 0 ? -B : B, a_y + (int64_t)dir * H, yt, s, ridx))) return rc;
       const char* ag = w.hp_dgt + (size_t)dir * 4 * H * (size_t)ceil_div(Mv, 32) * 128;
       if (grouped) {
         pr[npr++] = HpProblem{ag, a_dgc + (int64_t)dir * 4 * H, yt, a_y + (int64_t)dir * H, 4 * H, H, Mv, w.dwhh + (int64_t)dir * 4 * H * H, H, hpf};
         continue;
       }
-      if ((rc = hp_gemm(ag, a_dgc + (int64_t)dir * 4 * H, yt, a_y + (int64_t)dir * H, 4 * H, H, Mv, w.dwhh + (int64_t)dir * 4 * H * H, 1, H, 0,
-                        nullptr, hpf, w.scratch, w.scratch_bytes, s)))
+      const HpOutMap om = {nullptr, H, ngate};
+      if ((rc = hp_gemm(ag, a_dgc + (int64_t)dir * 4 * H, yt, a_y + (int64_t)dir * H, 4 * H, H, Mv, bd->dw_hh[dir], 1, H, 0,
+                        nullptr, hpf | accf, w.scratch, w.scratch_bytes, s, nullptr, 0, nullptr, &om)))
         return rc;
     }
+    dwhh_direct = !grouped;
     if (grouped) {
       if ((rc = hp_gemm_grouped(pr, npr, xcd_skip, reinterpret_cast<unsigned*>(w.scratch), (char*)w.scratch + HPQ_HEADER_BYTES,
                                 w.scratch_bytes - HPQ_HEADER_BYTES, s, k.status)))
@@ -1947,7 +1964,7 @@
       RNNT_CHECK_HIP(hipMemsetAsync(g.C, 0, (size_t)4 * H * H * 4, s));
     }
   }
-  {
+  if (!dwhh_direct) {
     const long per = (long)4 * H * H;
     hipLaunchKernelGGL(unpermute_w_kernel, dim3((unsigned)ceil_div(per, 256), D), dim3(256), 0, s, w.dwhh, H, H, per, ngate,
                        bd->dw_hh[0], D > 1 ? bd->dw_hh[1] : bd->dw_hh[0], acc);
@@ -1985,6 +2002,24 @@
   return lstm_bwd_impl(bd, precision, stream);
 }
 
+extern "C" int rnnt_hip_lstm_gate_permute(const float* w0, const float* w1, int32_t H, int64_t I, int32_t D, int32_t ngate, float* out, void* stream) {
+  RNNT_CHECK_ARG(w0 && out && H >= 1 && I >= 1 && I < (1ll << 31) / (4 * (int64_t)H) && (D == 1 || (D == 2 && w1)) && ngate >= 1 && ngate <= 4, "lstm_gate_permute: bad arguments");
+  const long per = (long)4 * H * I;
+  hipLaunchKernelGGL(permute_w_kernel, dim3((unsigned)ceil_div(per, 256), D), dim3(256), 0, (hipStream_t)stream, w0, D > 1 ? w1 : w0, (int)H, (int)I,
+                     (int)ngate, out);
+  RNNT_CHECK_LAUNCH();
+  return RNNT_OK;
+}
+extern "C" int rnnt_hip_lstm_gate_unpermute(const float* in, int32_t H, int64_t I, int32_t D, int32_t ngate, float* o0, float* o1, int32_t accumulate,
+                                            void* stream) {
+  RNNT_CHECK_ARG(in && o0 && H >= 1 && I >= 1 && I < (1ll << 31) / (4 * (int64_t)H) && (D == 1 || (D == 2 && o1)) && ngate >= 1 && ngate <= 4, "lstm_gate_unpermute: bad arguments");
+  const long per = (long)4 * H * I;
+  hipLaunchKernelGGL(unpermute_w_kernel, dim3((unsigned)ceil_div(per, 256), D), dim3(256), 0, (hipStream_t)stream, in, (int)H, (int)I, per, (int)ngate,
+                     o0, D > 1 ? o1 : o0, accumulate ? 1 : 0);
+  RNNT_CHECK_LAUNCH();
+  return RNNT_OK;
+}
+
 extern "C" int rnnt_hip_lstm_check(const void* workspace, void* stream) {
   RNNT_CHECK_ARG(workspace != nullptr, "lstm_check: null workspace");
   unsigned st = 0;
```

Result: faster. 1305 (median of 6 runs) (+1.2%).
